# anrieff/fray

Measured on AMD Instinct MI355X. Metric: Mrays/s (closest-hit + shadow rays) at 1920x1080, 64spp path trace, higher is better.
Workload: dtype f64

## Files before the change

### fray_amd/abi.py

```python
import ctypes as C

i32, u32, i64, u64, f32, f64 = C.c_int32, C.c_uint32, C.c_int64, C.c_uint64, C.c_float, C.c_double
P = C.POINTER

ABI_VERSION = 3

OK, E_ARG, E_PARSE, E_NODEVICE, E_UNSUPPORTED, E_NOMEM, E_HIP, E_CANCELLED = 0, -1, -2, -3, -4, -5, -6, -7
GEOM_PLANE, GEOM_SPHERE, GEOM_CUBE, GEOM_MESH, GEOM_CSG = range(5)
TEX_CHECKER, TEX_BITMAP, TEX_BUMP, TEX_FRESNEL = range(4)
SHADER_CONST, SHADER_LAMBERT, SHADER_PHONG, SHADER_REFL, SHADER_REFR, SHADER_LAYERED = range(6)
LIGHT_POINT, LIGHT_RECT = range(2)
MODE_PRIMARY_ID, MODE_RENDER = 0, 1
FRAME_STATS = 1
OPTION_NAMES = ("pt_lanes", "pt_budget_mib", "speculate_fans", "fused_whitted_max", "fp_contract", "seed_table_mib", "skip_null_segments",
                "segment_planes", "certified_segments")
FIGURE_NAMES = ("contracted_launches", "shadow_segments", "segment_plane_nodes", "certified_segments_eligible", "shadow_segments_certified",
                "shadow_nodes_skipped", "seed_table_bytes", "seed_launches", "seed_planes_reused", "batch_lanes", "whitted_path",
                "pt_budget_effective_mib", "scene_updates", "scene_update_bytes", "arena_bytes", "fans_filed", "fan_children",
                "fan_children_looked_up", "fans_given_up")


class Transform(C.Structure):
    _fields_ = [("offset", f64 * 3), ("m", f64 * 9), ("invM", f64 * 9)]

# ... 137 lines not shown
    _fields_ = [("seed", u32), ("spp", i32), ("sample_first", i32), ("rng_skip", i32), ("flags", i32), ("_pad", i32),
                ("keys", C.c_void_p)]


class Adaptive(C.Structure):
    _fields_ = [("min_spp", i32), ("_pad", i32), ("threshold", f64), ("err_floor", f64), ("rungs", i32), ("_pad2", i32),
                ("samples", u64)]


ACCUM_CHANNELS = 4


class Samples(C.Structure):
    _fields_ = [("sample_first", i32), ("sample_count", i32), ("samples_done", i32), ("_pad", i32)]


class SamplesMap(C.Structure):
    _fields_ = [("samples", u64), ("count_min", i32), ("count_max", i32)]


class SampleMap(C.Structure):
    _fields_ = [("tolerance", C.c_float), ("lum_floor", C.c_float), ("min_count", i32), ("max_count", i32), ("max_add", i32), ("grow", i32),
                ("pixels", u64), ("samples", u64)]


class Denoise(C.Structure):
    _fields_ = [("levels", i32), ("demodulate", i32), ("sigma_luminance", C.c_float), ("sigma_normal", C.c_float),
                ("sigma_depth", C.c_float), ("sigma_albedo", C.c_float)]


FEAT_CHANNELS = 10
MOTION_CHANNELS = 8


class View(C.Structure):
    _fields_ = [("pos", f32 * 3), ("right", f32 * 3), ("up", f32 * 3), ("front", f32 * 3), ("tan_x", C.c_float), ("tan_y", C.c_float),
                ("width", i32), ("height", i32)]


class Temporal(C.Structure):
    _fields_ = [("demodulate", i32), ("max_history", i32), ("variance_history", i32), ("alpha_min", C.c_float), ("film_offset", C.c_float),
                ("plane_tolerance", C.c_float), ("normal_min_dot", C.c_float)]


class Change(C.Structure):
    _fields_ = [("radius", i32), ("gain", C.c_float)]


HISTORY_CHANNELS = 12
HISTORY_SPLIT_CHANNELS = 20


STRUCTS = {"frayhip_transform": Transform, "frayhip_geom_ref": GeomRef, "frayhip_node": Node,
           "frayhip_plane": Plane, "frayhip_sphere": Sphere, "frayhip_cube": Cube,
           "frayhip_csg": Csg, "frayhip_triangle": Triangle, "frayhip_kdnode": KDNode,
           "frayhip_mesh": Mesh, "frayhip_texture": Texture, "frayhip_shader": Shader,
           "frayhip_layer": Layer, "frayhip_light": Light, "frayhip_camera": Camera,
           "frayhip_settings": Settings, "frayhip_environment": Environment,
           "frayhip_scene_desc": SceneDesc, "frayhip_frame": Frame, "frayhip_stats": Stats,
           "frayhip_progress": Progress, "frayhip_progressive": Progressive,
           "frayhip_shade_request": ShadeRequest, "frayhip_adaptive": Adaptive, "frayhip_samples": Samples,
           "frayhip_view": View, "frayhip_samples_map": SamplesMap}

VP = C.c_void_p
SYMBOLS = {
    "frayhip_scene_parse": (C.c_int, [C.c_char_p, P(VP)]),
    "frayhip_host_scene_desc": (P(SceneDesc), [VP]),
    "frayhip_host_scene_free": (None, [VP]),
    "frayhip_init": (C.c_int, [C.c_int]),
    "frayhip_scene_create": (C.c_int, [P(SceneDesc), P(VP)]),
    "frayhip_scene_destroy": (None, [VP]),
    "frayhip_scene_set_view": (C.c_int, [VP, P(Camera), P(Settings)]),
    "frayhip_scene_update": (C.c_int, [VP, P(SceneDesc)]),
    "frayhip_transform_identity": (C.c_int, [P(Transform)]),
    "frayhip_transform_scale": (C.c_int, [P(Transform), f64, f64, f64]),
    "frayhip_transform_rotate": (C.c_int, [P(Transform), f64, f64, f64]),
    "frayhip_transform_translate": (C.c_int, [P(Transform), f64, f64, f64]),
    "frayhip_light_begin_frame": (C.c_int, [P(Light)]),
    "frayhip_shader_begin_frame": (C.c_int, [P(Shader)]),
    "frayhip_scene_set_option": (C.c_int, [VP, C.c_char_p, i64]),
    "frayhip_scene_get_option": (C.c_int, [VP, C.c_char_p, P(i64)]),
    "frayhip_scene_tight_gates": (C.c_int, [VP, C.c_int, P(i64), P(i64)]),
    "frayhip_scene_camera_skip": (C.c_int, [VP, C.c_int, P(i64), P(i64), P(i64), P(i64)]),
    "frayhip_render": (C.c_int, [VP, P(Frame), VP, VP, VP, P(Stats)]),
    "frayhip_render_device": (C.c_int, [VP, P(Frame), VP, VP, VP, VP, P(Stats)]),
    "frayhip_render_progressive": (C.c_int, [VP, P(Frame), P(Progressive), VP, VP, VP, P(Stats)]),
    "frayhip_render_device_progressive": (C.c_int, [VP, P(Frame), P(Progressive), VP, VP, VP, VP, P(Stats)]),
    "frayhip_render_adaptive": (C.c_int, [VP, P(Frame), P(Adaptive), VP, VP, VP, P(Stats)]),
    "frayhip_render_device_adaptive": (C.c_int, [VP, P(Frame), P(Adaptive), VP, VP, VP, VP, P(Stats)]),
    "frayhip_render_samples": (C.c_int, [VP, P(Frame), P(Samples), P(Progressive), VP, VP, VP, P(Stats)]),
    "frayhip_render_samples_device": (C.c_int, [VP, P(Frame), P(Samples), P(Progressive), VP, VP, VP, VP, P(Stats)]),
    "frayhip_render_components": (C.c_int, [VP, P(Frame), P(Samples), P(Progressive), VP, VP, VP, VP, VP, VP, P(Stats)]),
    "frayhip_render_components_device": (C.c_int, [VP, P(Frame), P(Samples), P(Progressive), VP, VP, VP, VP, VP, VP, VP, P(Stats)]),
    "frayhip_render_samples_map": (C.c_int, [VP, P(Frame), P(SamplesMap), VP, VP, VP, VP, VP, P(Stats)]),
    "frayhip_render_samples_map_device": (C.c_int, [VP, P(Frame), P(SamplesMap), VP, VP, VP, VP, VP, VP, P(Stats)]),
    "frayhip_render_components_map": (C.c_int, [VP, P(Frame), P(SamplesMap), VP, VP, VP, VP, VP, VP, VP, VP, P(Stats)]),
    "frayhip_render_components_map_device": (C.c_int, [VP, P(Frame), P(SamplesMap), VP, VP, VP, VP, VP, VP, VP, VP, VP, P(Stats)]),
    "frayhip_sample_map_defaults": (C.c_int, [P(SampleMap)]),
    "frayhip_sample_map": (C.c_int, [C.c_int, C.c_int, VP, VP, P(SampleMap), VP, P(Stats)]),
    "frayhip_sample_map_device": (C.c_int, [C.c_int, C.c_int, VP, VP, P(SampleMap), VP, VP, P(Stats)]),
    "frayhip_sample_map_pair": (C.c_int, [C.c_int, C.c_int, VP, VP, VP, P(SampleMap), VP, P(Stats)]),
    "frayhip_sample_map_pair_device": (C.c_int, [C.c_int, C.c_int, VP, VP, VP, P(SampleMap), VP, VP, P(Stats)]),
    "frayhip_render_features": (C.c_int, [VP, P(Frame), C.c_int, VP, P(Stats)]),
    "frayhip_render_features_device": (C.c_int, [VP, P(Frame), C.c_int, VP, VP, P(Stats)]),
    "frayhip_render_features_motion": (C.c_int, [VP, P(Frame), C.c_int, P(Transform), C.c_int, VP, VP, P(Stats)]),
    "frayhip_render_features_motion_device": (C.c_int, [VP, P(Frame), C.c_int, P(Transform), C.c_int, VP, VP, VP, P(Stats)]),
    "frayhip_denoise_defaults": (C.c_int, [P(Denoise)]),
    "frayhip_denoise": (C.c_int, [C.c_int, C.c_int, VP, VP, VP, P(Denoise), VP, P(Stats)]),
    "frayhip_denoise_device": (C.c_int, [C.c_int, C.c_int, VP, VP, VP, P(Denoise), VP, VP, P(Stats)]),
    "frayhip_denoise_signal": (C.c_int, [C.c_int, C.c_int, VP, VP, VP, P(Denoise), VP, P(Stats)]),
    "frayhip_denoise_signal_device": (C.c_int, [C.c_int, C.c_int, VP, VP, VP, P(Denoise), VP, VP, P(Stats)]),
    "frayhip_view_from_camera": (C.c_int, [P(Camera), C.c_int, C.c_int, P(View)]),
    "frayhip_temporal_defaults": (C.c_int, [P(Temporal)]),
    "frayhip_temporal_accumulate": (C.c_int, [C.c_int, C.c_int, VP, VP, P(View), VP, P(Temporal), VP, VP, VP, P(Stats)]),
    "frayhip_temporal_accumulate_device": (C.c_int, [C.c_int, C.c_int, VP, VP, P(View), VP, P(Temporal), VP, VP, VP, VP, P(Stats)]),
    "frayhip_temporal_accumulate_motion": (C.c_int, [C.c_int, C.c_int, VP, VP, VP, P(View), VP, P(Temporal), VP, VP, VP, P(Stats)]),
    "frayhip_temporal_accumulate_motion_device": (C.c_int, [C.c_int, C.c_int, VP, VP, VP, P(View), VP, P(Temporal), VP, VP, VP, VP, P(Stats)]),
    "frayhip_temporal_accumulate_split": (C.c_int, [C.c_int, C.c_int, VP, VP, VP, VP, P(View), VP, P(Temporal), P(Temporal), VP, VP, VP, VP, VP, P(Stats)]),
    "frayhip_temporal_accumulate_split_device": (C.c_int, [C.c_int, C.c_int, VP, VP, VP, VP, P(View), VP, P(Temporal), P(Temporal), VP, VP, VP, VP, VP, VP,
                                                           P(Stats)]),
    "frayhip_change_defaults": (C.c_int, [P(Change)]),
    "frayhip_change_frame": (C.c_int, [C.c_int, C.c_int, VP, VP, VP, P(Change), VP, P(Stats)]),
    "frayhip_change_frame_device": (C.c_int, [C.c_int, C.c_int, VP, VP, VP, P(Change), VP, VP, P(Stats)]),
    "frayhip_temporal_accumulate_adaptive": (C.c_int, [C.c_int, C.c_int, VP, VP, VP, VP, P(View), VP, P(Temporal), VP, VP, VP, P(Stats)]),
    "frayhip_temporal_accumulate_adaptive_device": (C.c_int, [C.c_int, C.c_int, VP, VP, VP, VP, P(View), VP, P(Temporal), VP, VP, VP, VP, P(Stats)]),
    "frayhip_temporal_accumulate_split_adaptive": (C.c_int, [C.c_int, C.c_int, VP, VP, VP, VP, VP, VP, P(View), VP, P(Temporal), P(Temporal), VP, VP, VP, VP,
                                                             VP, P(Stats)]),
    "frayhip_temporal_accumulate_split_adaptive_device": (C.c_int, [C.c_int, C.c_int, VP, VP, VP, VP, VP, VP, P(View), VP, P(Temporal), P(Temporal), VP, VP,
                                                                    VP, VP, VP, VP, P(Stats)]),
    "frayhip_camera_rays": (C.c_int, [VP, i64, VP, C.c_int, VP, VP]),
    "frayhip_camera_rays_device": (C.c_int, [VP, i64, VP, C.c_int, VP, VP, VP]),
    "frayhip_trace_rays": (C.c_int, [VP, i64, VP, VP, C.c_int, VP, VP, VP, P(Stats)]),
    "frayhip_trace_rays_device": (C.c_int, [VP, i64, VP, VP, C.c_int, VP, VP, VP, VP, P(Stats)]),
    "frayhip_visible": (C.c_int, [VP, i64, VP, VP, C.c_int, VP, P(Stats)]),
    "frayhip_visible_device": (C.c_int, [VP, i64, VP, VP, C.c_int, VP, VP, P(Stats)]),
    "frayhip_shade_rays": (C.c_int, [VP, i64, VP, VP, P(ShadeRequest), VP, P(Stats)]),
    "frayhip_shade_rays_device": (C.c_int, [VP, i64, VP, VP, P(ShadeRequest), VP, VP, P(Stats)]),
    "frayhip_bucket_count": (C.c_int, [C.c_int, C.c_int, C.c_int, C.c_int]),
    "frayhip_pack_buckets_device": (C.c_int, [VP, VP, C.c_int, C.c_int, C.c_int, C.c_int, C.c_int, VP]),
    "frayhip_unpack_buckets_device": (C.c_int, [VP, VP, C.c_int, C.c_int, C.c_int, C.c_int, C.c_int, VP]),
    "frayhip_bucket_xy": (C.c_int, [C.c_int, C.c_int, C.c_int, C.POINTER(C.c_int), C.POINTER(C.c_int)]),
    "frayhip_comm_available": (C.c_int, []),
    "frayhip_comm_library": (C.c_char_p, []),
    "frayhip_comm_unique_id": (C.c_int, [VP]),
    "frayhip_comm_create": (C.c_int, [VP, C.c_int, C.c_int, P(VP)]),
    "frayhip_comm_from_nccl": (C.c_int, [VP, C.c_int, C.c_int, P(VP)]),
    "frayhip_comm_ranks": (C.c_int, [VP]),
    "frayhip_comm_destroy": (None, [VP]),
    "frayhip_gather_buckets": (C.c_int, [VP, VP, C.c_int, C.c_int, C.c_int, C.c_int, VP]),
    "frayhip_to_rgb32": (C.c_int, [VP, VP, C.c_int]),
    "frayhip_save_bmp": (C.c_int, [C.c_char_p, VP, C.c_int, C.c_int]),
    "frayhip_debug_rng": (C.c_int, [u32, C.c_int, VP, VP, VP, C.c_int]),
    "frayhip_debug_libm": (C.c_int, [C.c_int, VP, VP, VP, VP, VP]),
    "frayhip_debug_arith": (C.c_int, [C.c_int, C.c_int, VP, VP, VP]),
    "frayhip_last_error": (C.c_char_p, []),
    "frayhip_abi_version": (C.c_int, []),
    "frayhip_sizeof": (C.c_int, [C.c_char_p]),
}


def bind(lib):
    for name, (res, args) in SYMBOLS.items():
        fn = getattr(lib, name)
        fn.restype = res
        fn.argtypes = args
    return lib
# ... 1 lines not shown
```

### fray_amd/csrc/capi.hip

```cpp
#include <hip/hip_runtime.h>

#include <algorithm>
#include <chrono>
#include <cstddef>
#include <cmath>
#include <cstring>
#include <string>
#include <vector>
#include <functional>
#include <cstdlib>


#include "entry_support.hpp"
#include "dev_rng.hpp"
#include "dev_pack.hpp"
#include "scene_arena.hpp"

namespace {

using frayhip_detail::set_error;

void put3(double* o, const double* p) { o[0] = p[0]; o[1] = p[1]; o[2] = p[2]; }
}

// ... 148 lines not shown
    if (T.d) (void)hipFree(T.d);
    T.d = nullptr;
    T.bytes = 0;
    T.valid.clear();
    T.serving = false;
}

void seed_table_begin(frayhip_scene* sc, const DFrame& F, int nItems, int spp)
{
    SeedTable& T = sc->seedTab;
    if (!sc->seedTableCapBytes) { seed_table_free(sc); T.keyed = false; return; }
    if (nItems <= 0 || spp <= 0) return;
    const int32_t key[7] = {F.W, F.H, F.BW, F.BH, F.bucketFirst, F.bucketStride, F.nBuckets};
    const size_t planeBytes = (size_t)nItems * sizeof(uint32_t);
    if (!T.keyed || memcmp(key, T.key, sizeof key) != 0 || F.seed != T.seed || nItems != T.nItems) {
        memcpy(T.key, key, sizeof key);
        T.seed = F.seed; T.nItems = nItems; T.keyed = true; T.noGrow = false;
        T.valid.assign(T.bytes / planeBytes, 0);
    }
    const size_t need = (size_t)spp * planeBytes;
    if (need > sc->seedTableCapBytes) return;
    if (T.valid.size() < (size_t)spp) {
        if (T.noGrow) return;
        uint32_t* d = nullptr;
        if (hipMalloc((void**)&d, need) != hipSuccess) {
            (void)hipGetLastError();
            seed_table_free(sc);
            T.noGrow = true;
            return;
        }
        size_t held = 0;
        for (size_t s = 0; s < T.valid.size(); s++) if (T.valid[s]) held = s + 1;
        if (held && hipMemcpy(d, T.d, held * planeBytes, hipMemcpyDeviceToDevice) != hipSuccess) { (void)hipGetLastError(); std::fill(T.valid.begin(), T.valid.end(), (unsigned char)0); }
        if (T.d) (void)hipFree(T.d);
        T.d = d;
        T.bytes = need;
        T.valid.resize((size_t)spp, 0);
    }
    T.serving = true;
}

hipEvent_t pool_event(std::vector<hipEvent_t>& pool, size_t i)
{
    while (pool.size() <= i) {
        hipEvent_t e = nullptr;
        hipError_t rc = hipEventCreate(&e);
        if (rc != hipSuccess) { set_error(std::string("hipEventCreate: ") + hipGetErrorString(rc)); return nullptr; }
        pool.push_back(e);
    }
    return pool[i];
}

int bad(const char* who, const std::string& why)
{
    set_error(std::string(who) + ": " + why);
    return FRAYHIP_E_ARG;
}
int unsupported(const char* who, const std::string& why)
{
    set_error(std::string(who) + ": " + why);
    return FRAYHIP_E_UNSUPPORTED;
}

int frame_spp(const frayhip_scene* s)
{
    int spp = s->settings.wantAA ? 5 : 1;
    if (s->camera.dof) spp = std::max(spp, s->camera.numDOFSamples);
    if (s->settings.gi) spp = std::max(spp, s->settings.numPaths);
    return spp;
}

DScene frame_scene(const frayhip_scene* s)
{
    const frayhip_settings& set = s->settings;
    DScene S = s->S;
    S.ambient[0] = set.ambientLight[0]; S.ambient[1] = set.ambientLight[1]; S.ambient[2] = set.ambientLight[2];
    S.maxTraceDepth = set.maxTraceDepth;
    S.gi = set.gi;
    S.saturation = set.saturation;
    S.skipNullSegments = s->skipNullSegments ? 1 : 0;
    S.segmentPlanes = s->segmentPlanes ? 1 : 0;
    S.certifiedSegments = (s->certifiedSegments && s->segmentPlanes && S.segCertAll) ? 1 : 0;
    if (!s->cameraSkip) S.nCamSkip = 0;
    return S;
}

DFrame frame_record(const frayhip_scene* s, int bucketFirst, int bucketStride, uint32_t seed)
{
    DFrame F = frame_grid(s->settings.frameWidth, s->settings.frameHeight);
    F.bucketStride = bucketStride > 0 ? bucketStride : 1;
    F.bucketFirst = bucketFirst;
    F.nBuckets = frayhip_bucket_count(F.W, F.H, F.bucketFirst, F.bucketStride);
    F.spp = frame_spp(s);
    F.seed = seed;
    F.jitter = (s->camera.dof || s->settings.gi) ? 1 : 0;
    return F;
}

int check_bucket_range(const char* who, int nBuckets) { return nBuckets < 0 ? bad(who, "bad bucket_first / bucket_stride") : FRAYHIP_OK; }
int check_pixel_cap(const char* who, int nBuckets)
{
    if ((long long)nBuckets * 2304 > (1ll << 30)) return unsupported(who, "more than 2^30 pixels in one call (shard the frame with bucket_first / bucket_stride)");
    return FRAYHIP_OK;
}
int refuse_stereo(const char* who, const frayhip_scene* s) { return s->camera.stereoSeparation > 0 ? unsupported(who, "stereo frames are not supported") : FRAYHIP_OK; }
int refuse_long_generators(const char* who, const frayhip_scene* s, const char* by)
{
    if (s->settings.gi && s->settings.maxTraceDepth >= 0 && long_generators(s->settings.maxTraceDepth))
        return unsupported(who, std::string("path tracing with maxTraceDepth >= 20 (generators past 227 words) is not supported by ") + by);
    return FRAYHIP_OK;
}

frayhip_stats finish_stats(frayhip_scene* sc, const DStats* blocks, int nBlocks, size_t nTraceEvents, size_t nShadowEvents, std::chrono::steady_clock::time_point t0)
{
    frayhip_stats o{};
    for (int k = 0; k < nBlocks; k++) {
        const DStats& d = blocks[k];
        o.closest_rays += d.closest; o.shadow_rays += d.shadow; o.node_tests += d.node; o.kd_inner_visits += d.kdInner; o.leaf_refs += d.leafRefs;
        o.tri_tests += d.tri; o.prim_tests += d.prim; o.smooth_hits += d.smooth; o.samples += d.samples; o.texture_fetches += d.tex;
    }
    float ms = 0;
    (void)hipEventElapsedTime(&ms, sc->evA, sc->evB);
    o.ms_kernels = ms;
    auto sumEvents = [](const std::vector<hipEvent_t>& pool, size_t n) {
        double t = 0;
        for (size_t i = 0; i + 1 < n; i += 2) {
            float m2 = 0;
            (void)hipEventElapsedTime(&m2, pool[i], pool[i + 1]);
            t += m2;
        }
        return t;
    };
    o.ms_trace = sumEvents(sc->evPool, nTraceEvents);
    o.trace_launches = nTraceEvents / 2;
    o.ms_shadow = sumEvents(sc->evPoolShadow, nShadowEvents);
    o.shadow_launches = nShadowEvents / 2;
    o.ms_total = std::chrono::duration<double, std::milli>(std::chrono::steady_clock::now() - t0).count();
    return o;
}

}

struct SceneEdit {
    frayhip_arena::ArenaFacts F;
    std::vector<frayhip_arena::ArenaTable> tables;
    std::vector<frayhip_arena::ArenaMeshTables> meshTables;
    std::vector<int64_t> texelOffset;
    std::vector<unsigned char> host;
    std::vector<int64_t> hostOff;
    int32_t counts[11];
    int64_t nTexels;
    std::vector<frayhip_geom_ref> geoms;
    std::vector<frayhip_csg> csgs;
    std::vector<frayhip_mesh> meshes;
    std::vector<frayhip_texture> textures;
    frayhip_environment environment;
};

namespace frayhip_detail {
const DNode* host_nodes(const frayhip_scene* s) { return (const DNode*)(s->edit->host.data() + s->edit->hostOff[s->edit->F.tNodes]); }
}

namespace {

using frayhip_detail::kStatsBytes;
using frayhip_detail::grid_for;
// ... 168 lines not shown
    sc->whittedNeedsRecursion = F.whittedNeedsRecursion != 0;
    sc->lightDraws = F.lightDraws != 0;
    sc->lightSampleCount = F.lightSampleCount;
    sc->specFanMax = F.specFanMax;
}

}

extern "C" {

int frayhip_init(int device_id)
{
    int n = 0;
    hipError_t e = hipGetDeviceCount(&n);
    if (e != hipSuccess || n <= 0) { set_error("frayhip_init: no HIP device available"); return FRAYHIP_E_NODEVICE; }
    if (device_id < 0 || device_id >= n) { set_error("frayhip_init: bad device id"); return FRAYHIP_E_ARG; }
    HIP_TRY(hipSetDevice(device_id));
    return FRAYHIP_OK;
}

int frayhip_scene_create(const frayhip_scene_desc* desc, frayhip_scene** out)
{
    if (!desc || !out) { set_error("frayhip_scene_create: null argument"); return FRAYHIP_E_ARG; }
    if (desc->abi_version != FRAYHIP_ABI_VERSION) { set_error("frayhip_scene_create: ABI version mismatch"); return FRAYHIP_E_ARG; }
    const frayhip_scene_desc& d = *desc;
    {
        const std::string why = validate_desc(d);
        if (!why.empty()) { set_error(why); return FRAYHIP_E_ARG; }
    }
    {
        std::vector<int> levels(d.n_csgs, 0);
        std::function<int(int, int)> depth = [&](int i, int guard) -> int {
            if (guard > d.n_csgs) return 1 << 20;
            if (levels[i]) return levels[i];
            int m = 1;
            for (int side = 0; side < 2; side++) {
                const frayhip_geom_ref& g = d.geoms[side == 0 ? d.csgs[i].left : d.csgs[i].right];
                if (g.kind == FRAYHIP_GEOM_CSG) m = std::max(m, 1 + depth(g.index, guard + 1));
            }
            return levels[i] = m;
        };
        for (int i = 0; i < d.n_csgs; i++)
            if (depth(i, 0) > FRAY_CSG_DEPTH) {
                set_error("frayhip_scene_create: CSG operands nested more than " + std::to_string(FRAY_CSG_DEPTH) + " levels deep are not implemented on the device path");
                return FRAYHIP_E_UNSUPPORTED;
            }
    }
    frayhip_arena::ArenaBuilt B;
    frayhip_arena::arena_build(d, B);
    frayhip_scene* sc = new frayhip_scene();
    commit_facts(sc, B.F);
    if (hipMalloc(&sc->d_arena, B.host.size() ? B.host.size() : 256) != hipSuccess) {
        set_error("frayhip_scene_create: hipMalloc failed (no device?)");
        delete sc;
        return FRAYHIP_E_NODEVICE;
    }
    {
        unsigned char* const base = (unsigned char*)sc->d_arena;
        std::vector<unsigned char*> stage(B.tables.size());
        std::vector<const unsigned char*> addr(B.tables.size());
        for (size_t t = 0; t < B.tables.size(); t++) { stage[t] = B.host.data() + B.tables[t].off; addr[t] = base + B.tables[t].off; }
        frayhip_arena::arena_place(B.F, B.meshTables.data(), B.texelOffset.data(), stage.data(), addr.data(), sc->S);
    }
    hipError_t e = hipMemcpy(sc->d_arena, B.host.data(), B.host.size(), hipMemcpyHostToDevice);
    if (e != hipSuccess) { set_error(std::string("frayhip_scene_create: upload failed: ") + hipGetErrorString(e)); (void)hipFree(sc->d_arena); delete sc; return FRAYHIP_E_NODEVICE; }
    sc->arena_bytes = B.host.size();
    sc->edit = make_scene_edit(d, B);
    sc->camera = d.camera;
    sc->settings = d.settings;
    if (hipMalloc((void**)&sc->d_stats, kStatsBytes) != hipSuccess || hipMalloc((void**)&sc->d_qmeta, 3 * FRAY_PT_LANES * sizeof(QMeta)) != hipSuccess ||
        hipEventCreate(&sc->evA) != hipSuccess || hipEventCreate(&sc->evB) != hipSuccess || !create_lanes(sc)) {
        set_error("frayhip_scene_create: could not allocate the per-scene device state");
        frayhip_scene_destroy(sc);
        return FRAYHIP_E_NOMEM;
    }
    if (const char* e = getenv("FRAYHIP_PT_LANES")) { long v = atol(e); if (v >= 1 && v <= FRAY_PT_LANES) sc->ptLanes = (int)v; }
    if (const char* e = getenv("FRAYHIP_SPECULATE_FANS")) sc->speculateFans = atol(e) != 0;
    if (const char* e = getenv("FRAYHIP_FP_CONTRACT")) sc->fpContract = atol(e) == 1;
    if (const char* e = getenv("FRAYHIP_SKIP_NULL_SEGMENTS")) sc->skipNullSegments = atol(e) != 0;
    if (const char* e = getenv("FRAYHIP_SEGMENT_PLANES")) sc->segmentPlanes = atol(e) != 0;
    if (const char* e = getenv("FRAYHIP_CERTIFIED_SEGMENTS")) sc->certifiedSegments = atol(e) != 0;
    if (const char* e = getenv("FRAYHIP_TIGHT_GATES")) sc->tightGates = atol(e) != 0;
    if (const char* e = getenv("FRAYHIP_CAMERA_SKIP")) sc->cameraSkip = atol(e) != 0;
    if (const char* e = getenv("FRAYHIP_FUSED_WHITTED_MAX")) { long v = atol(e); if (v >= 0 && v <= 1024) sc->fusedWhittedMax = (int)v; }
    if (const char* e = getenv("FRAYHIP_CSG_LANES")) { long v = atol(e); if (v >= 1 && v <= FRAY_PT_LANES) sc->csgLanes = (int)v; }
    if (const char* e = getenv("FRAYHIP_SEED_TABLE_MIB")) { long v = atol(e); if (v >= 0 && v <= (1 << 20)) sc->seedTableCapBytes = (size_t)v << 20; }
    if (const char* e = getenv("FRAYHIP_PT_BUDGET_MIB")) { long v = atol(e); if (v >= 1 && v <= (1 << 20)) { sc->ptBudgetBytes = (size_t)v << 20; sc->ptBudgetEff = 0; } }
    *out = sc;
    return FRAYHIP_OK;
}

int frayhip_scene_get_option(frayhip_scene* s, const char* name, int64_t* value)
{
    if (!s || !name || !value) { set_error("frayhip_scene_get_option: null argument"); return FRAYHIP_E_ARG; }
    const std::string n(name);
    if (n == "pt_lanes") *value = s->ptLanes;
    else if (n == "pt_budget_mib") *value = (int64_t)(s->ptBudgetBytes >> 20);
    else if (n == "speculate_fans") *value = s->speculateFans ? 1 : 0;
    else if (n == "fp_contract") *value = s->fpContract ? 1 : 0;
    else if (n == "contracted_launches") *value = s->lastContracted;
    else if (n == "skip_null_segments") *value = s->skipNullSegments ? 1 : 0;
    else if (n == "shadow_segments") *value = s->lastShadowSegments;
    else if (n == "segment_planes") *value = s->segmentPlanes ? 1 : 0;
    else if (n == "segment_plane_nodes") *value = s->S.nSegNodes;
    else if (n == "certified_segments") *value = s->certifiedSegments ? 1 : 0;
    else if (n == "certified_segments_eligible") *value = s->S.segCertAll;
    else if (n == "shadow_segments_certified") *value = s->lastShadowCertified;
    else if (n == "shadow_nodes_skipped") *value = s->lastShadowNodesSkipped;
    else if (n == "seed_table_mib") *value = (int64_t)(s->seedTableCapBytes >> 20);
    else if (n == "seed_table_bytes") *value = (int64_t)s->seedTab.bytes;
    else if (n == "seed_launches") *value = s->lastSeedLaunches;
    else if (n == "seed_planes_reused") *value = s->lastSeedReused;
    else if (n == "batch_lanes") *value = s->lastBatchLanes;
    else if (n == "whitted_path") *value = s->lastWhittedPath;
    else if (n == "fused_whitted_max") *value = s->fusedWhittedMax;
    else if (n == "pt_budget_effective_mib") *value = (int64_t)(frayhip_detail::work_budget(s) >> 20);
    else if (n == "scene_updates") *value = s->sceneUpdates;
    else if (n == "scene_update_bytes") *value = s->sceneUpdateBytes;
    else if (n == "arena_bytes") *value = (int64_t)s->arena_bytes;
    else if (n == "fans_filed") *value = s->lastFans[0];
    else if (n == "fan_children") *value = s->lastFans[1];
    else if (n == "fan_children_looked_up") *value = s->lastFans[2];
    else if (n == "fans_given_up") *value = s->lastFans[3];
    else { set_error("frayhip_scene_get_option: unknown option " + n); return FRAYHIP_E_ARG; }
    return FRAYHIP_OK;
}

int frayhip_scene_set_option(frayhip_scene* s, const char* name, int64_t value)
{
    if (!s || !name) { set_error("frayhip_scene_set_option: null argument"); return FRAYHIP_E_ARG; }
    if (s->rendering) { set_error("frayhip_scene_set_option: the scene is rendering a frame"); return FRAYHIP_E_ARG; }
    const std::string n(name);
    if (n == "pt_lanes") {
        if (value < 1 || value > FRAY_PT_LANES) { set_error("frayhip_scene_set_option: pt_lanes must be 1.." + std::to_string(FRAY_PT_LANES)); return FRAYHIP_E_ARG; }
        s->ptLanes = (int)value;
    } else if (n == "pt_budget_mib") {
        if (value < 1 || value > (1 << 20)) { set_error("frayhip_scene_set_option: pt_budget_mib must be 1..1048576"); return FRAYHIP_E_ARG; }
        s->ptBudgetBytes = (size_t)value << 20;
        s->ptBudgetEff = 0;
    } else if (n == "speculate_fans") {
        if (value != 0 && value != 1) { set_error("frayhip_scene_set_option: speculate_fans must be 0 or 1"); return FRAYHIP_E_ARG; }
        s->speculateFans = value != 0;
    } else if (n == "fused_whitted_max") {
        if (value < 0 || value > 1024) { set_error("frayhip_scene_set_option: fused_whitted_max must be 0..1024"); return FRAYHIP_E_ARG; }
        s->fusedWhittedMax = (int)value;
    } else if (n == "fp_contract") {
        if (value != 0 && value != 1) { set_error("frayhip_scene_set_option: fp_contract must be 0 or 1"); return FRAYHIP_E_ARG; }
        s->fpContract = value != 0;
    } else if (n == "seed_table_mib") {
        if (value < 0 || value > (1 << 20)) { set_error("frayhip_scene_set_option: seed_table_mib must be 0..1048576"); return FRAYHIP_E_ARG; }
        s->seedTableCapBytes = (size_t)value << 20;
        if (s->seedTab.bytes > s->seedTableCapBytes) { frayhip_detail::seed_table_free(s); s->seedTab.keyed = false; }
    } else if (n == "skip_null_segments") {
        if (value != 0 && value != 1) { set_error("frayhip_scene_set_option: skip_null_segments must be 0 or 1"); return FRAYHIP_E_ARG; }
        s->skipNullSegments = value != 0;
    } else if (n == "segment_planes") {
        if (value != 0 && value != 1) { set_error("frayhip_scene_set_option: segment_planes must be 0 or 1"); return FRAYHIP_E_ARG; }
        s->segmentPlanes = value != 0;
    } else if (n == "certified_segments") {
        if (value != 0 && value != 1) { set_error("frayhip_scene_set_option: certified_segments must be 0 or 1"); return FRAYHIP_E_ARG; }
        s->certifiedSegments = value != 0;
    } else {
        set_error("frayhip_scene_set_option: unknown option " + n);
        return FRAYHIP_E_ARG;
    }
    return FRAYHIP_OK;
}

int frayhip_scene_tight_gates(frayhip_scene* s, int enable, int64_t* enabled, int64_t* eligible)
{
    if (!s) { set_error("frayhip_scene_tight_gates: null scene"); return FRAYHIP_E_ARG; }
    if (enable < -1 || enable > 1) { set_error("frayhip_scene_tight_gates: enable must be -1, 0 or 1"); return FRAYHIP_E_ARG; }
    if (enable >= 0 && s->rendering) { set_error("frayhip_scene_tight_gates: the scene is rendering a frame"); return FRAYHIP_E_ARG; }
    if (enable >= 0) s->tightGates = enable != 0;
    if (enabled) *enabled = s->tightGates ? 1 : 0;
    if (eligible) *eligible = s->edit->F.nTightGates;
    return FRAYHIP_OK;
}

int frayhip_scene_camera_skip(frayhip_scene* s, int enable, int64_t* enabled, int64_t* eligible, int64_t* skipped, int64_t* waves)
{
    if (!s) { set_error("frayhip_scene_camera_skip: null scene"); return FRAYHIP_E_ARG; }
    if (enable < -1 || enable > 1) { set_error("frayhip_scene_camera_skip: enable must be -1, 0 or 1"); return FRAYHIP_E_ARG; }
    if (enable >= 0 && s->rendering) { set_error("frayhip_scene_camera_skip: the scene is rendering a frame"); return FRAYHIP_E_ARG; }
    if (enable >= 0) s->cameraSkip = enable != 0;
    if (enabled) *enabled = s->cameraSkip ? 1 : 0;
    if (eligible) *eligible = s->edit->F.nCamSkip;
    if (skipped) *skipped = s->lastCameraSkipped;
    if (waves) *waves = s->lastCameraWaves;
    return FRAYHIP_OK;
}

int frayhip_scene_set_view(frayhip_scene* s, const frayhip_camera* camera, const frayhip_settings* settings)
{
    if (!s) { set_error("frayhip_scene_set_view: null scene"); return FRAYHIP_E_ARG; }
    if (s->rendering) { set_error("frayhip_scene_set_view: the scene is rendering a frame"); return FRAYHIP_E_ARG; }
    if (settings && (settings->frameWidth <= 0 || settings->frameHeight <= 0)) { set_error("frayhip_scene_set_view: bad frame size"); return FRAYHIP_E_ARG; }
    if (camera) s->camera = *camera;
    if (settings) s->settings = *settings;
    return FRAYHIP_OK;
}

int frayhip_scene_update(frayhip_scene* s, const frayhip_scene_desc* desc)
{
    if (!s || !desc) { set_error("frayhip_scene_update: null argument"); return FRAYHIP_E_ARG; }
    if (s->rendering) { set_error("frayhip_scene_update: the scene is rendering a frame"); return FRAYHIP_E_ARG; }
    if (desc->abi_version != FRAYHIP_ABI_VERSION) { set_error("frayhip_scene_update: ABI version mismatch"); return FRAYHIP_E_ARG; }
    const frayhip_scene_desc& d = *desc;
    SceneEdit& E = *s->edit;
    if (const char* what = fixed_part_differs(E, d)) {
        set_error(std::string("frayhip_scene_update: ") + what + " differs from the description the scene was created from (only nodes, primitives, shaders, layers, lights and texture parameters can be edited)");
        return FRAYHIP_E_ARG;
    }
    {
        const std::string why = validate_editable(d, "frayhip_scene_update");
        if (!why.empty()) { set_error(why); return FRAYHIP_E_ARG; }
    }
    std::vector<unsigned char> next(E.host);
    frayhip_arena::ArenaFacts F = E.F;
    std::vector<unsigned char*> tab(E.tables.size());
    std::vector<const unsigned char*> addr(E.tables.size());
    for (size_t t = 0; t < E.tables.size(); t++) {
        tab[t] = E.hostOff[t] >= 0 ? next.data() + E.hostOff[t] : nullptr;
        addr[t] = (const unsigned char*)s->d_arena + E.tables[t].off;
    }
    frayhip_arena::arena_update(d, E.meshTables.data(), F, tab.data());
    DScene S = s->S;
    frayhip_arena::arena_place(F, E.meshTables.data(), E.texelOffset.data(), tab.data(), addr.data(), S);
    long long bytes = 0;
    for (int32_t t : frayhip_arena::arena_editable_tables(F)) {
        if (!E.tables[t].bytes) continue;
        HIP_TRY(hipMemcpy((unsigned char*)s->d_arena + E.tables[t].off, tab[t], E.tables[t].bytes, hipMemcpyHostToDevice));
        bytes += (long long)E.tables[t].bytes;
    }
    E.host.swap(next);
    E.F = F;
    commit_facts(s, F);
    s->S = S;
    s->sceneUpdates++;
    s->sceneUpdateBytes = bytes;
    return FRAYHIP_OK;
}

void frayhip_scene_destroy(frayhip_scene* s)
{
    if (!s) return;
    delete s->edit;
    if (s->d_arena) (void)hipFree(s->d_arena);
    if (s->d_work) (void)hipFree(s->d_work);
    frayhip_detail::seed_table_free(s);
    if (s->d_stats) (void)hipFree(s->d_stats);
    if (s->d_motionTab) (void)hipFree(s->d_motionTab);
    if (s->d_qmeta) (void)hipFree(s->d_qmeta);
    if (s->evA) (void)hipEventDestroy(s->evA);
    if (s->evB) (void)hipEventDestroy(s->evB);
    if (s->evLaneStart) (void)hipEventDestroy(s->evLaneStart);
    for (int k = 0; k < FRAY_PT_LANES; k++) {
        if (s->evResolved[k]) (void)hipEventDestroy(s->evResolved[k]);
        if (s->laneStream[k]) (void)hipStreamDestroy(s->laneStream[k]);
    }
    for (auto e : s->evPool) (void)hipEventDestroy(e);
    for (auto e : s->evPoolShadow) (void)hipEventDestroy(e);
    delete s;
}


namespace {
int render_dispatch(frayhip_scene* s, const frayhip_frame* f, float* d_rgb, int32_t* d_hit_id, double* d_hit_dist, hipStream_t stream, frayhip_stats* st,
                    const frayhip_detail::Progress* prog)
{
    if (s->rendering) { set_error("frayhip_render: the scene is already rendering a frame (a render call from inside a progress callback?)"); return FRAYHIP_E_ARG; }
    frayhip_detail::Busy busy(s, stream, false);
    return frayhip_detail::for_flag_word(frayhip_detail::flag_word(s, (f->flags & FRAYHIP_FRAME_STATS) != 0), [&](auto w) {
        return frayhip_detail::render_impl<decltype(w)::value>(s, f, d_rgb, d_hit_id, d_hit_dist, stream, st, prog, nullptr);
    });
// ... 153 lines not shown
```

### fray_amd/csrc/dev_scene.hpp

```cpp
#pragma once
#include <stdint.h>
#include "frayhip.h"
#include "dev_tricert.hpp"
#include "dev_segcert.hpp"
#include "dev_gatecert.hpp"

#ifdef __HIP_DEVICE_COMPILE__
#define FRAY_RO __attribute__((address_space(4)))
#else
#define FRAY_RO
#endif

#define FRAY_CSG_MAX 30
#ifndef FRAY_CSG_DEPTH
#define FRAY_CSG_DEPTH 16
#endif

#define FRAY_KD_LDS_STACK 16
#define FRAY_KD_MAX_DEPTH 72

struct DXform { double off[3]; double m[9]; double inv[9]; };

struct DTri;
struct DNode {
    DXform T;
    int32_t geomKind, geomIndex, shader, bumpTex;
    int32_t xfClass;
    int32_t tlTris;
    int32_t tlCulling;
    int32_t xfIdentity;
    double bmin[3], bmax[3];
    const FRAY_RO DTri* tlPtr;
    double boxMax;
    int32_t gated;
    int32_t segNode;
};
struct DNodeX {
    double bminE[3], bmaxE[3];
    double cc[3], ch[3], cM;
    int32_t csgBox, padX;
};

struct DPlane { double limit, height; };
struct DSphere { double O[3]; double R; };
struct DCube { double O[3]; double halfSide; };
struct DCsg { int32_t op, leftKind, leftIndex, rightKind, rightIndex, leftGeom, rightGeom, flat; };

struct DTri {
    double g[3];
    double A[3];
    double N[3];
    double AC[3];
    double AB[3];
    int32_t index;
    int32_t pad;
};

struct DTriAttr {
    double nA[3], nB[3], nC[3];
    double tA[2], tB[2], tC[2];
    double dNdx[3], dNdy[3];
};

struct alignas(16) DKd {
    union {
        double split;
        struct { int32_t triBegin, triCount; };
    };
    int32_t child0;
    int32_t meta;
};
struct DKdBox { double lo[3], hi[3]; };

struct DMesh {
    double bmin[3], bmax[3];
    const FRAY_RO DTri* tris;
    const FRAY_RO DTriAttr* attrs;
    const FRAY_RO DKd* kd;
    const FRAY_RO DKdBox* kdBox;
    const FRAY_RO int32_t* refs;
    const FRAY_RO DTri* ltris;
    int32_t nTris, hasKd, smooth, culling, hasUV, pad;
    double boxMax;
    const FRAY_RO DTri32* ltris32;
    double ref[3];
};

struct DTexture {
    int32_t kind, width, height, pad;
    float color1[3], color2[3];
    double scaling, bumpIntensity, ior;
    const FRAY_RO float* texels;
};

struct DShader {
    int32_t kind, texture;
    float color[3], specularColor[3], mult[3];
    int32_t numSamples;
    double exponent, specularMultiplier, glossiness, deflectionScaling, ior;
    int32_t layerBegin, layerCount;
    int32_t usesUV, pad;
};

struct DLayer { int32_t shader, texture; float opacity[3]; int32_t pad; };

struct DLight {
    int32_t kind, xSubd, ySubd, pad;
    float color[3], power;
    double pos[3];
    DXform T;
    double center[3];
    double area;
    double areaXsize, areaYsize;
};

struct DEnv {
    int32_t present, loaded;
    int32_t width[6], height[6];
    const FRAY_RO float* face[6];
};

struct DCamera {
    double topLeft[3], topRight[3], bottomLeft[3];
    double frontDir[3], upDir[3], rightDir[3], pos[3];
    double w, h, apertureSize, focalPlaneDist, stereoSeparation;
    float leftMask[3], rightMask[3];
    int32_t dof, pad;
};

#define FRAY_MAX_GATES 8
#define FRAY_GATE_MIN_TRIS 6
struct DGate { double lo[3], hi[3]; float cf[3], hf[3]; float Mf; int32_t exact; float guard; int32_t nDirs; float nf[FRAY_GATE_MAX_DIRS][3]; };

#define FRAY_CAMSKIP_MAX 16
struct DCamSkip { float cf[3], hf[3]; float Mf, guard; float nf[FRAY_GATE_MAX_DIRS][3]; int32_t nDirs, node; };

struct DScene {
    const FRAY_RO DNode* nodes;
    const FRAY_RO DNodeX* nodesX;
    const FRAY_RO DGate* gates;
    int32_t nGates, gatesExact;
    const FRAY_RO DPlane* planes;
    const FRAY_RO DSphere* spheres;
    const FRAY_RO DCube* cubes;
    const FRAY_RO DCsg* csgs;
    const FRAY_RO DMesh* meshes;
    const FRAY_RO DShader* shaders;
    const FRAY_RO DLayer* layers;
    const FRAY_RO DTexture* textures;
    const FRAY_RO DLight* lights;
    DEnv env;
    int32_t nNodes, nLights;
    float probPickLight;
    float ambient[3];
    int32_t maxTraceDepth, gi;
    float saturation;
    const FRAY_RO DSegPlane* segPlanes;
    const FRAY_RO uint32_t* segNodeMasks;
    int32_t nSegPlanes, nSegNodes;
    int32_t segmentPlanes;
    int32_t skipNullSegments;
    int32_t segCertAll;
    int32_t certifiedSegments;
    const FRAY_RO DCamSkip* camSkip;
    int32_t nCamSkip, padCamSkip;
};

struct DFrame {
    int32_t W, H, BW, BH;
    int32_t bucketFirst, bucketStride, nBuckets , spp;
    uint32_t seed;
    int32_t jitter;
};

struct DStats {
    unsigned long long closest, shadow, node, kdInner, leafRefs, tri, prim, smooth, samples, tex, rngOverflow;
#ifdef FRAY_STAMPS
    unsigned long long stamp[24];
    unsigned long long stampLanes[24];
#endif
};
struct DCursors { unsigned int v[8][32]; };
```

### fray_amd/csrc/dev_shade.hpp

```cpp
#pragma once
#include "dev_math.hpp"
#include "dev_rng.hpp"
#include "dev_scene.hpp"
#include "dev_trace.hpp"

enum { RF_DIFFUSE = 2 };

struct HitInfo {
    V3 ip, norm, dNdx, dNdy;
    double u, v;
};

FD void prim_attributes(const DScene& S, int kind, int index, V3 ipl, int code, double l2, double l3, bool needUV, bool needBump, V3& nl, HitInfo& info)
{
    if (kind == 0) {
        nl = v3(0, 1, 0);
        info.u = ipl.x;
        info.v = ipl.z;
    } else if (kind == 1) {
        const FRAY_RO DSphere& Sp = S.spheres[index];
        nl = normalized(ipl - ld3(Sp.O));
        if (needUV) {
            info.u = ((atan2(nl.z, nl.x) / FRAY_PI * 180.0) + 180.0) / 360.0;
            info.v = 1 - ((asin(nl.y) / FRAY_PI * 180.0) + 90) / 180.0;
        }
    } else if (kind == 2) {
        const int ax = code >> 1;
        const double sg = (code & 1) ? +1.0 : -1.0;
        nl = v3(ax == 0 ? sg : 0.0, ax == 1 ? sg : 0.0, ax == 2 ? sg : 0.0);
        if (ax == 0) { info.u = ipl.y; info.v = ipl.z; }
        else if (ax == 1) { info.u = ipl.x; info.v = ipl.z; }
        else { info.u = ipl.x; info.v = ipl.y; }
    } else {
        const FRAY_RO DMesh& M = S.meshes[index];
        const FRAY_RO DTriAttr* A = M.attrs + code;
        if (M.smooth) {
            V3 nA = ld3(A->nA), nB = ld3(A->nB), nC = ld3(A->nC);
            nl = normalized(nA + (nB - nA) * l2 + (nC - nA) * l3);
        } else {
            nl = ld3(M.tris[code].g);
        }
        if (M.hasUV) {
            info.u = A->tA[0] + (A->tB[0] - A->tA[0]) * l2 + (A->tC[0] - A->tA[0]) * l3;
            info.v = A->tA[1] + (A->tB[1] - A->tA[1]) * l2 + (A->tC[1] - A->tA[1]) * l3;
        }
        if (needBump) {
            info.dNdx = ld3(A->dNdx);
            info.dNdy = ld3(A->dNdy);
        }
    }
}

template <int ST, bool BARY = false, bool ANY_UV = false>
FD void finalize_hit(const DScene& S, const HitT<ST>& h, V3 o, V3 d, bool needUV, HitInfo& info)
{
    const FRAY_RO DNode& N = S.nodes[h.node];
    needUV = needUV && (ANY_UV || tex_variant(ST));
    const bool needBump = tex_variant(ST) && N.bumpTex >= 0;
    V3 ls = mulM(o - ld3(N.T.off), N.T.inv);
    V3 ldir = normalized(mulM(d, N.T.inv));
    V3 ipl = ls + ldir * h.t;
    V3 nl;
    info.dNdx = v3(0, 0, 0);
    info.dNdy = v3(0, 0, 0);
    info.u = 0; info.v = 0;
    bool done = false;
    if constexpr ((ST & 2) != 0) {
        if (N.geomKind == 2) {
            ipl = h.ipl;
            prim_attributes(S, 2, N.geomIndex, ipl, h.tri, 0, 0, needUV, needBump, nl, info);
            done = true;
        } else if (N.geomKind == 4) {
            ipl = h.ipl;
            prim_attributes(S, h.leafKind, h.leafIndex, ipl, h.tri, h.l2, h.l3, needUV, needBump, nl, info);
            done = true;
        }
    }
    if (!done) {
        double l2 = h.l2, l3 = h.l3;
        if (BARY && N.geomKind == 3) {
            const FRAY_RO DMesh& M = S.meshes[N.geomIndex];
            if (M.smooth || M.hasUV) tri_bary(M.tris + h.tri, ls, ldir, l2, l3);
        }
        prim_attributes(S, N.geomKind, N.geomIndex, ipl, h.tri, l2, l3, needUV, needBump, nl, info);
    }
    info.ip = mulM(ipl, N.T.m) + ld3(N.T.off);
    info.norm = normalized(mulM(nl, N.T.m));
}

template <int ST>
FD C3 texel(const FRAY_RO DTexture& T, int x, int y, Cnt& c)
{
    bump<ST>(c.tex);
    if (T.width <= 0 || x < 0 || x >= T.width || y < 0 || y >= T.height) return c3(0, 0, 0);
    return ldc(T.texels + 3 * ((long long)x + (long long)y * T.width));
}
FD void wrap_texel(const FRAY_RO DTexture& T, double u, double v, int& ix, int& iy)
{
    ix = int(floor(u * T.scaling * T.width));
    iy = int(floor(v * T.scaling * T.height));
    ix %= T.width;
    iy %= T.height;
    if (ix < 0) ix += T.width;
    if (iy < 0) iy += T.height;
}
FD float fresnel_schlick(V3 i, V3 n, float ior)
{
    float q = (1.0f - ior) / (1.0f + ior);
    float f = (float)((double)q * (double)q);
    float NdotI = (float)-dot(n, i);
    return f + (1.0f - f) * powf(1.0f - NdotI, 5.0f);
}
template <int ST>
FD C3 texture_sample(const DScene& S, int t, V3 rayDir, const HitInfo& info, Cnt& c)
{
    if (!tex_variant(ST)) return c3(1, 1, 1);
    const FRAY_RO DTexture& T = S.textures[t];
    if (T.kind == 0) {
        int ix = int(floor(info.u * T.scaling) / 5.0);
        int iy = int(floor(info.v * T.scaling) / 5.0);
        return ((ix + iy) % 2 == 0) ? ldc(T.color1) : ldc(T.color2);
    }
    if (T.kind == 1) {
        int ix, iy;
        wrap_texel(T, info.u, info.v, ix, iy);
        return texel<ST>(T, ix, iy, c);
    }
    if (T.kind == 3) {
        V3 n;
        double myIor;
        if (dot(rayDir, info.norm) < 0) { n = info.norm; myIor = T.ior; }
        else { n = -info.norm; myIor = 1.0 / T.ior; }
        float f = fresnel_schlick(rayDir, n, (float)myIor);
        return c3(f, f, f);
    }
    return c3(0, 0, 0);
}
template <int ST>
FD void apply_bump(const DScene& S, int nodeIdx, HitInfo& info, Cnt& c)
{
    if (!tex_variant(ST)) return;
    int bt = S.nodes[nodeIdx].bumpTex;
    if (bt < 0) return;
    const FRAY_RO DTexture& T = S.textures[bt];
    if (T.kind != 2) return;
    int ix, iy;
    wrap_texel(T, info.u, info.v, ix, iy);
    C3 t = texel<ST>(T, ix, iy, c);
    float dx = (float)(t.r * T.bumpIntensity);
    float dy = (float)(t.g * T.bumpIntensity);
    info.norm = info.norm + ((double)dx * info.dNdx + (double)dy * info.dNdy) * T.bumpIntensity;
    info.norm = normalized(info.norm);
}

template <int ST>
FD C3 environment(const DScene& S, V3 dir, Cnt& c)
{
    if (!tex_variant(ST) || !S.env.present || !S.env.loaded) return c3(0, 0, 0);
    double maxVal = fabs(dir.x);
    int dim = 0;
    if (fabs(dir.y) > maxVal) { dim = 1; maxVal = fabs(dir.y); }
    if (fabs(dir.z) > maxVal) dim = 2;
    bool positive = comp(dir, dim) > 0;
    V3 on = dir * (1.0 / fabs(comp(dir, dim)));
    int face = (positive ? 3 : 0) + dim;
    double sx, sy;
    switch (face) {
        case 0: sx = on.z; sy = -on.y; break;
        case 3: sx = -on.z; sy = -on.y; break;
        case 1: sx = on.x; sy = -on.z; break;
        case 4: sx = on.x; sy = on.z; break;
        case 2: sx = on.x; sy = on.y; break;
        default: sx = on.x; sy = -on.y; break;
    }
    int W = S.env.width[face], H = S.env.height[face];
    int ix = (int)(((sx + 1) / 2) * W);
    int iy = (int)(((sy + 1) / 2) * H);
    bump<ST>(c.tex);
    if (ix < 0 || ix >= W || iy < 0 || iy >= H) return c3(0, 0, 0);
    return ldc(S.env.face[face] + 3 * ((long long)ix + (long long)iy * W));
}

FD int light_num_samples(const FRAY_RO DLight& L) { return L.kind == 0 ? 1 : L.xSubd * L.ySubd; }
FD C3 light_color(const FRAY_RO DLight& L) { return ldc(L.color) * L.power; }
template <class G>
FD void light_nth_sample(const FRAY_RO DLight& L, int idx, V3 shadePos, G& tab, V3& samplePos, C3& color)
{
    if (L.kind == 0) {
        samplePos = ld3(L.pos);
        color = ldc(L.color) * L.power;
        return;
    }
    int col = idx % L.xSubd;
    int row = idx / L.xSubd;
    double cellW = L.areaXsize;
    double cellH = L.areaYsize;
    double x0 = col * cellW;
    double y0 = row * cellH;
    double p_x = x0 + cellW * rng_float(tab);
    double p_y = y0 + cellH * rng_float(tab);
    V3 pl = v3(p_x - 0.5, 0, p_y - 0.5);
    V3 sp = mulM(shadePos - ld3(L.T.off), L.T.inv);
    if (sp.y > 0) {
        color = c3(0, 0, 0);
    } else {
        float cw = float(fray_div(dot(v3(0, -1, 0), sp), length(sp)));
        color = ldc(L.color) * L.power * (float)L.area * cw;
    }
    samplePos = mulM(pl, L.T.m) + ld3(L.T.off);
}
FD double light_solid_angle(const FRAY_RO DLight& L, V3 ip)
{
    if (L.kind == 0) return 0;
    double q = lengthSqr(ip - ld3(L.center));
    return fray_div(L.area, 1.0 < q ? q : 1.0);
}

template <int ST, class G>
FD C3 shade_direct(const DScene& S, const FRAY_RO DShader& sh, V3 rayDir, const HitInfo& info, G& tab, bool phong, Cnt& c)
{
    C3 diffuse = ldc(sh.color);
    if (sh.texture >= 0) diffuse = diffuse * texture_sample<ST>(S, sh.texture, rayDir, info, c);
    C3 result = diffuse * ldc(S.ambient);
    const int nl = S.nLights;
    for (int li = 0; li < nl; li++) {
        const FRAY_RO DLight& L = S.lights[li];
        const int ns = light_num_samples(L);
        C3 sum = c3(0, 0, 0);
        for (int k = 0; k < ns; k++) {
            C3 lc;
            V3 lp;
            light_nth_sample(L, k, info.ip, tab, lp, lc);
            double d2 = lengthSqr(info.ip - lp);
            V3 wl = normalized(lp - info.ip);
            V3 n = faceforward(rayDir, info.norm);
            float cosN = (float)dot(wl, n);
            float lam = (float)(cosN / d2);
            lam = lam > 0.0f ? lam : 0.0f;
            if (visible<ST>(S, info.ip + n * 1e-6, lp, c)) {
                C3 r = diffuse * lc * lam;
                if (phong) {
                    V3 wi = -wl;
                    V3 rr = reflect(wi, n);
                    double cosV = dot(-rayDir, rr);
                    if (cosV > 0)
                        r = r + lc / (float)d2 * ldc(sh.specularColor) * (float)pow(cosV, sh.exponent) * (float)sh.specularMultiplier;
                }
                sum = sum + r;
            }
        }
        result = result + sum / (float)ns;
    }
    return result;
}

template <class G>
FD V3 hemisphere_sample(G& tab, V3 norm)
{
    double u = rng_double(tab);
    double v = rng_double(tab);
    double theta = 2 * FRAY_PI * u;
    double sp, cp, st, ct;
    fray_acos_sincos(2 * v - 1, &sp, &cp);
    fray_sincos(theta, &st, &ct);
    V3 dir = v3(sp * ct, cp, sp * st);
    if (dot(dir, norm) > 0) return dir;
    return -dir;
}
FD C3 brdf_eval(const FRAY_RO DShader& sh, const HitInfo& x, V3 w_out)
{
    if (sh.kind == 1) {
        double dd = dot(x.norm, w_out);
        float cosTerm = (float)(0.0 < dd ? dd : 0.0);
        return ldc(sh.color) * (float)fray_div(cosTerm, FRAY_PI);
    }
    if (sh.kind == 3 || sh.kind == 4) return c3(0, 0, 0);
    return c3(1, 0, 0);
}
FD int spawn_words(const FRAY_RO DShader& sh) { return sh.kind == 1 ? 4 : 0; }

struct PathRay { V3 o, d; int depth; unsigned flags; };

template <class G>
FD void spawn_ray(const FRAY_RO DShader& sh, const HitInfo& x, const PathRay& w_in, G& tab, PathRay& w_out, C3& brdf, float& pdf)
{
    w_out = w_in;
    if (sh.kind == 1) {
        w_out.depth = w_in.depth + 1;
        w_out.o = x.ip + x.norm * 1e-6;
        w_out.d = hemisphere_sample(tab, x.norm);
        w_out.flags |= RF_DIFFUSE;
        double dd = dot(x.norm, w_out.d);
        float cosTerm = (float)(0.0 < dd ? dd : 0.0);
        brdf = ldc(sh.color) * (float)fray_div(cosTerm, FRAY_PI);
        pdf = (float)(1 / (2 * FRAY_PI));
        return;
    }
    if (sh.kind == 3) {
        V3 n = faceforward(w_in.d, x.norm);
        w_out.depth = w_in.depth + 1;
        w_out.o = x.ip + n * 1e-6;
        w_out.d = reflect(w_in.d, x.norm);
        w_out.flags &= ~(unsigned)RF_DIFFUSE;
        brdf = ldc(sh.mult) * 1e9f;
        pdf = 1e9f;
        return;
    }
    if (sh.kind == 4) {
        V3 n = faceforward(w_in.d, x.norm);
        double myIor = dot(n, x.norm) > 0 ? 1.0 / sh.ior : sh.ior / 1.0;
        V3 refr = refract(w_in.d, n, myIor);
        if (!(refr.x == 0 && refr.y == 0 && refr.z == 0)) {
            w_out.o = x.ip - n * 1e-6;
            w_out.d = refr;
            w_out.depth = w_in.depth + 1;
            w_out.flags &= ~(unsigned)RF_DIFFUSE;
            brdf = ldc(sh.mult) * 1e9f;
            pdf = 1e9f;
        } else {
            w_out.depth = w_in.depth + 1;
            brdf = c3(0, 0, 0);
            pdf = 1.0f;
        }
        return;
    }
    w_out.depth = w_in.depth + 1;
    brdf = c3(1, 0, 0);
    pdf = 1;
}

template <class GR, class GT>
FD bool nee_prepare(const DScene& S, V3 rayDir, const HitInfo& info, C3 pm, const FRAY_RO DShader& sh, GR& rnd, GT& tab, V3& a, V3& b, C3& contrib, bool skipNull)
{
    if (S.nLights == 0) return false;
    int lightIdx = rng_int0(rnd, S.nLights - 1);
    const FRAY_RO DLight& L = S.lights[lightIdx];
    V3 x = info.ip;
    double solidAngle = light_solid_angle(L, x);
    if (solidAngle == 0) return false;
    int randSample = rng_int0(rnd, light_num_samples(L) - 1);
    V3 pl;
    C3 unused;
    light_nth_sample(L, randSample, x, tab, pl, unused);
    if (skipNull && (sh.kind == 3 || sh.kind == 4)) return false;
    a = x + info.norm * 1e-6;
    b = pl;
    C3 Le = light_color(L);
    V3 w_out = normalized(pl - x);
    C3 brdfAtPoint = brdf_eval(sh, info, w_out);
    if (intensity(brdfAtPoint) == 0) { contrib = c3(0, 0, 0); return !skipNull; }
    float probHitLightArea = (float)fray_rcp(solidAngle);
    float probPickThisLight = S.probPickLight;
    float chooseLightProb = probHitLightArea * probPickThisLight;
    contrib = Le * pm * brdfAtPoint / chooseLightProb;
    if (skipNull && (__float_as_uint(contrib.r) | __float_as_uint(contrib.g) | __float_as_uint(contrib.b)) == 0u) return false;
    return true;
}
```

### fray_amd/csrc/dev_trace.hpp

```cpp
#pragma once
#ifndef FRAY_IDENTITY_SKIP
#define FRAY_IDENTITY_SKIP 1
#endif
#ifndef FRAY_FILTER_STRAIGHT
#define FRAY_FILTER_STRAIGHT 1
#endif
#include "dev_math.hpp"
#include "dev_scene.hpp"
#include "dev_sort.hpp"
#define FRAY_CERT_SEQ() __builtin_amdgcn_sched_barrier(0)
#include "dev_boxcert.hpp"
#include "dev_misscert.hpp"
#include "dev_segcert.hpp"

#ifdef FRAY_LEAFSTAT
static __device__ unsigned long long g_leafStat[4];
#endif
struct Cnt {
    unsigned long long closest, shadow, node, kdInner, leafRefs, tri, prim, smooth, samples, tex;
    unsigned envelope;
};
template <int ST> FD void bump(unsigned long long& c, unsigned long long n = 1) { if (ST & 1) c += n; }
constexpr bool kd_variant(int st) { return (st & 6) != 0; }
constexpr bool tex_variant(int st) { return (st & 14) != 0; }
constexpr bool identity_variant(int st) { return FRAY_IDENTITY_SKIP && (st & 14) == 0; }
constexpr bool tight_variant(int st) { return FRAY_ARITH == 0 && (st & 15) == 0; }

struct HitRec {
    int node;
    int tri;
    double dist;
    double t;
    double l2, l3;
};
struct HitRecX : HitRec {
    V3 ipl;
    int leafKind, leafIndex;
};
template <int ST> struct HitOf { typedef HitRec type; };
template <> struct HitOf<2> { typedef HitRecX type; };
template <> struct HitOf<3> { typedef HitRecX type; };
template <int ST> using HitT = typename HitOf<ST>::type;

struct Box6 { double lox, loy, loz, hix, hiy, hiz; };

struct LocalRay { V3 s, d, rd; int cls; bool haveRd, dirOk; double rmax, sMax; };


FD bool box_inside(const Box6& b, V3 v)
{
    return b.lox - 1e-6 <= v.x && v.x <= b.hix + 1e-6 && b.loy - 1e-6 <= v.y && v.y <= b.hiy + 1e-6 &&
           b.loz - 1e-6 <= v.z && v.z <= b.hiz + 1e-6;
}

struct BoxDim { bool rej, hit; };
FD BoxDim box_dim(double sd, double dd, double rd, double lo, double hi, double su, double du, double lou, double hiu,
                  double sv, double dv, double lov, double hiv)
{
    BoxDim r;
    r.rej = (dd < 0 && sd < lo) | (dd > 0 && sd > hi);
    const bool skip = fabs(dd) < 1e-9;
    const double d1 = (lo - sd) * rd;
    const bool near = !(d1 < 0);
    const double x1 = su + du * d1, y1 = sv + dv * d1;
    const bool hitN = (lou <= x1) & (x1 <= hiu) & (lov <= y1) & (y1 <= hiv);
    const double d2 = (hi - sd) * rd;
    const bool far = !(d2 < 0);
    const double x2 = su + du * d2, y2 = sv + dv * d2;
    const bool hitF = far & (lou <= x2) & (x2 <= hiu) & (lov <= y2) & (y2 <= hiv);
    r.hit = !r.rej & !skip & near & (hitN | hitF);
    return r;
}

FD bool box_test_pre(const Box6& b, const Box6& be, V3 s, V3 d, V3 rd)
{
    bool res = be.lox <= s.x && s.x <= be.hix && be.loy <= s.y && s.y <= be.hiy && be.loz <= s.z && s.z <= be.hiz;
    bool alive = !res;
    if (!__any(alive)) return res;
    BoxDim a = box_dim(s.x, d.x, rd.x, b.lox, b.hix, s.y, d.y, b.loy, b.hiy, s.z, d.z, b.loz, b.hiz);
    res |= alive & a.hit;
    alive &= !a.rej & !a.hit;
    if (!__any(alive)) return res;
    a = box_dim(s.y, d.y, rd.y, b.loy, b.hiy, s.x, d.x, b.lox, b.hix, s.z, d.z, b.loz, b.hiz);
    res |= alive & a.hit;
    alive &= !a.rej & !a.hit;
    if (!__any(alive)) return res;
    a = box_dim(s.z, d.z, rd.z, b.loz, b.hiz, s.x, d.x, b.lox, b.hix, s.y, d.y, b.loy, b.hiy);
    res |= alive & a.hit;
    return res;
}

FD bool box_test(const Box6& b, V3 s, V3 d, V3 rd)
{
    bool res = box_inside(b, s);
    bool alive = !res;
    BoxDim a = box_dim(s.x, d.x, rd.x, b.lox, b.hix, s.y, d.y, b.loy, b.hiy, s.z, d.z, b.loz, b.hiz);
    res |= alive & a.hit;
    alive &= !a.rej & !a.hit;
    if (!__any(alive)) return res;
    a = box_dim(s.y, d.y, rd.y, b.loy, b.hiy, s.x, d.x, b.lox, b.hix, s.z, d.z, b.loz, b.hiz);
    res |= alive & a.hit;
    alive &= !a.rej & !a.hit;
    if (!__any(alive)) return res;
    a = box_dim(s.z, d.z, rd.z, b.loz, b.hiz, s.x, d.x, b.lox, b.hix, s.y, d.y, b.loy, b.hiy);
    res |= alive & a.hit;
    return res;
}

FD void box_set_hi(Box6& b, int axis, double v) { b.hix = axis == 0 ? v : b.hix; b.hiy = axis == 1 ? v : b.hiy; b.hiz = axis == 2 ? v : b.hiz; }
// ... 653 lines not shown
        tri = h.code;
        t = h.dist;
        l2 = h.l2; l3 = h.l3;
        lo->kind = h.leafKind; lo->index = h.leafIndex;
        return true;
    }
    double gamma;
    if (N.tlTris > 0) {
        prepare_ray<ST>(lr);
        Box6 box;
        box.lox = N.bmin[0]; box.loy = N.bmin[1]; box.loz = N.bmin[2];
        box.hix = N.bmax[0]; box.hiy = N.bmax[1]; box.hiz = N.bmax[2];
        bool rootHit;
        if constexpr (kd_variant(ST)) {
            TState st;
            rootHit = box_test_cert(box, lr, cert_ray(lr.rmax, lr.sMax, lr.dirOk, N.boxMax), st);
        } else {
            const FRAY_RO DNodeX& X = S.nodesX[nodeIndex];
            Box6 be;
            be.lox = X.bminE[0]; be.loy = X.bminE[1]; be.loz = X.bminE[2];
            be.hix = X.bmaxE[0]; be.hiy = X.bmaxE[1]; be.hiz = X.bmaxE[2];
            rootHit = box_test_pre(box, be, ls, ld, lr.rd);
        }
        STAMP(2);
        if (!rootHit) return false;
        gamma = 1e99;
        bool found = false;
        const int n = N.tlTris, culling = N.tlCulling;
        const FRAY_RO DTri* tris = N.tlPtr;
        for (int i = 0; i < n; i++)
            if (tri_test<ST>(tris + i, culling, ls, ld, gamma, l2, l3, c)) { found = true; tri = i; }
        STAMP(3);
        if (!found) return false;
    } else if (!kd_variant(ST)) {
        return false;
    } else if (!mesh_intersect<ST>(S.meshes[N.geomIndex], lr, gamma, tri, l2, l3, c)) return false;
    ipl = ls + ld * gamma;
    t = gamma;
    return true;
}

template <int ST>
FD bool node_intersect(const DScene& S, int i, V3 o, V3 d, LocalRay& lr, double& dist, double& t, int& tri, double& l2, double& l3, V3* iplOut, LeafOut* lo, Cnt& c)
{
    bump<ST>(c.node);
    const FRAY_RO DNode& N = S.nodes[i];
    if (N.xfClass != lr.cls) {
        bool done = false;
        if constexpr (identity_variant(ST)) {
#if FRAY_ARITH
            if (N.xfIdentity) { lr.s = o; lr.d = d; done = true; }
#else
            const bool zeros = o.x == 0 || o.y == 0 || o.z == 0 || d.x == 0 || d.y == 0 || d.z == 0;
            if (N.xfIdentity && !__any(zeros)) { lr.s = o; lr.d = normalized(d); done = true; }
#endif
        }
        if (!done) {
            lr.s = mulM(o - ld3(N.T.off), N.T.inv);
            lr.d = normalized(mulM(d, N.T.inv));
        }
        lr.cls = N.xfClass;
        lr.haveRd = false;
    }
    STAMP(1);
    V3 ipl;
    const bool hit = geom_intersect<ST>(S, N, i, lr, ipl, t, tri, l2, l3, lo, c);
    STAMP(5);
    if (!hit) return false;
    if constexpr ((ST & 2) != 0) { if (iplOut) *iplOut = ipl; }
    V3 ipw;
    if constexpr (identity_variant(ST)) {
#if FRAY_ARITH
        if (N.xfIdentity) { dist = t; STAMP(6); return true; }
#endif
        ipw = N.xfIdentity ? ipl : mulM(ipl, N.T.m) + ld3(N.T.off);
    } else {
        ipw = mulM(ipl, N.T.m) + ld3(N.T.off);
    }
    dist = length(o - ipw);
    STAMP(6);
    return true;
}

template <int ST>
FD bool light_intersect(const FRAY_RO DLight& L, V3 o, V3 d, double& dist, Cnt& c)
{
    if (L.kind == 0) return false;
    bump<ST>(c.prim);
    V3 ls = mulM(o - ld3(L.T.off), L.T.inv);
    V3 ldir = normalized(mulM(d, L.T.inv));
    if (ls.y >= 0) return false;
    if (ldir.y <= 0) return false;
    double travelByY = fabs(ls.y);
    double unitTravel = fabs(ldir.y);
    double scaling = fray_div(travelByY, unitTravel);
    V3 ip = ls + ldir * scaling;
    if (fabs(ip.x) > 0.5 || fabs(ip.z) > 0.5) return false;
    ip = mulM(ip, L.T.m) + ld3(L.T.off);
    dist = length(o - ip);
    return true;
}

FD void light_record(const FRAY_RO DLight& L, V3 o, V3 d, V3& ip, V3& norm)
{
    V3 ls = mulM(o - ld3(L.T.off), L.T.inv);
    V3 ldir = normalized(mulM(d, L.T.inv));
    double scaling = fray_div(fabs(ls.y), fabs(ldir.y));
    ip = mulM(ls + ldir * scaling, L.T.m) + ld3(L.T.off);
    norm = normalized(mulM(v3(0, -1, 0), L.T.m));
}

template <int ST, bool CAMSKIP = false>
FD void closest_hit(const DScene& S, V3 o, V3 d, HitT<ST>& best, Cnt& c, bool gateFree = false, uint32_t skipNodes = 0u)
{
    bump<ST>(c.closest);
    best.node = -1;
    best.tri = -1;
    best.dist = 1e99;
    best.t = 0; best.l2 = 0; best.l3 = 0;
    const int nn = S.nNodes;
    LocalRay lr;
    lr.cls = -1;
    lr.haveRd = false;
    for (int i = 0; i < nn; i++) {
        double dist, t, l2 = 0, l3 = 0;
        int tri = -1;
        if constexpr (CAMSKIP) { if (i < 32 && ((skipNodes >> i) & 1u)) continue; }
        if constexpr (!(ST & 1)) { if (S.nodes[i].gated) { if (gateFree) continue; } }
        if constexpr ((ST & 2) != 0) {
            V3 ipl;
            LeafOut lo{0, 0};
            if (node_intersect<ST>(S, i, o, d, lr, dist, t, tri, l2, l3, &ipl, &lo, c) && dist < best.dist) {
                best.node = i; best.tri = tri; best.dist = dist; best.t = t; best.l2 = l2; best.l3 = l3;
                best.ipl = ipl; best.leafKind = lo.kind; best.leafIndex = lo.index;
            }
        } else if (node_intersect<ST>(S, i, o, d, lr, dist, t, tri, l2, l3, nullptr, nullptr, c) && dist < best.dist) {
            best.node = i; best.tri = tri; best.dist = dist; best.t = t; best.l2 = l2; best.l3 = l3;
        }
    }
    if ((ST & 1) && best.node >= 0) {
        const FRAY_RO DNode& W = S.nodes[best.node];
        if (W.geomKind == 3 && S.meshes[W.geomIndex].smooth) c.smooth++;
    }
    STAMP(6);
    const int nl = S.nLights;
    for (int i = 0; i < nl; i++) {
        double dist;
        if (light_intersect<ST>(S.lights[i], o, d, dist, c) && dist < best.dist) {
            best.node = -2 - i;
            best.dist = dist;
        }
    }
    STAMP(7);
}

FD uint32_t segment_skip_nodes(const DScene& S, V3 a, V3 b, bool live)
{
    const int nP = S.segmentPlanes ? S.nSegPlanes : 0;
    if (nP <= 0) return 0u;
    const V3 e = b - a;
    const double m = seg_cert_scale(a.x, a.y, a.z, b.x, b.y, b.z, e.x, e.y, e.z);
    const lanes_t all = lanes(true);
    uint32_t certified = 0;
    for (int p = 0; p < nP; p++) {
        const FRAY_RO DSegPlane& P = S.segPlanes[p];
        if (lanes(!live || seg_same_side(P.N[0], P.N[1], P.N[2], P.k, P.t0, P.t1, m, a.x, a.y, a.z, b.x, b.y, b.z)) == all) certified |= 1u << p;
    }
    uint32_t skipNodes = 0;
    const int nS = S.nSegNodes;
    for (int j = 0; j < nS; j++)
        if ((S.segNodeMasks[j] & ~certified) == 0u) skipNodes |= 1u << j;
    return skipNodes;
}

FD uint32_t camera_skip_nodes(const DScene& S, V3 o, V3 d, bool live)
{
    const int nR = S.nCamSkip;
    if (nR <= 0) return 0u;
    const float dx = (float)d.x, dy = (float)d.y, dz = (float)d.z;
    const float dsum = fabsf(dx) + fabsf(dy) + fabsf(dz);
    const float ox = (float)o.x, oy = (float)o.y, oz = (float)o.z;
    const float omax = fmaxf(fmaxf(fabsf(ox), fabsf(oy)), fabsf(oz));
    const bool range = gate_ray_range(dsum, omax, ox + oy + oz);
    const lanes_t all = lanes(true);
    uint32_t skipNodes = 0;
    for (int r = 0; r < nR; r++) {
        const FRAY_RO DCamSkip& R = S.camSkip[r];
        bool miss = ray_surely_misses_box_f32(R.cf[0], R.cf[1], R.cf[2], R.hf[0], R.hf[1], R.hf[2], R.Mf, ox, oy, oz, dx, dy, dz, omax, dsum);
        miss = miss & gate_guard_f32(R, dx, dy, dz, dsum);
        miss = miss & range;
        if (lanes(!live || miss) == all) skipNodes |= 1u << R.node;
    }
    return skipNodes;
}

#ifdef __HIP__
#define FRAY_RCPF(x) __builtin_amdgcn_rcpf(x)
#else
#define FRAY_RCPF(x) (1.0f / (x))
#endif
template <bool TIGHT = false>
FD uint32_t ray_gate_class(const DScene& S, V3 o, V3 d)
{
    const int ng = S.nGates;
    if (ng == 0) return 0u;
    if constexpr (TIGHT) {
        if (S.gatesExact) {
            const float dx = (float)d.x, dy = (float)d.y, dz = (float)d.z;
            const float dsum = fabsf(dx) + fabsf(dy) + fabsf(dz);
            bool guarded = true, tight = false;
            for (int g = 0; g < ng; g++) {
                const FRAY_RO DGate& G = S.gates[g];
                if (G.nDirs) { guarded = guarded & gate_guard_f32(G, dx, dy, dz, dsum); tight = true; }
            }
            FRAY_CERT_SEQ();
            const float ox = (float)o.x, oy = (float)o.y, oz = (float)o.z;
            const float omax = fmaxf(fmaxf(fabsf(ox), fabsf(oy)), fabsf(oz));
            uint32_t first = 0;
            for (int g = ng - 1; g >= 0; g--) {
                const FRAY_RO DGate& G = S.gates[g];
                if (!ray_surely_misses_box_f32(G.cf[0], G.cf[1], G.cf[2], G.hf[0], G.hf[1], G.hf[2], G.Mf, ox, oy, oz, dx, dy, dz, omax, dsum)) first = (uint32_t)g + 1u;
            }
            if (tight) guarded = guarded & gate_ray_range(dsum, omax, ox + oy + oz);
            if (!guarded && !first) first = 1u;
            return !(omax < 1e9f) && !first ? 1u : first;
        }
    }
    const float ox = (float)o.x, oy = (float)o.y, oz = (float)o.z;
    if (S.gatesExact) {
        const float dx = (float)d.x, dy = (float)d.y, dz = (float)d.z;
        const float omax = fmaxf(fmaxf(fabsf(ox), fabsf(oy)), fabsf(oz)), dsum = fabsf(dx) + fabsf(dy) + fabsf(dz);
// ... 60 lines not shown
```

### fray_amd/csrc/kernels.hpp

```cpp
#pragma once
#include "dev_shade.hpp"
#include "dev_whitted.hpp"
#include "dev_queues.hpp"
#include <type_traits>

#ifndef FRAY_PRIMARY_WAVES
#define FRAY_PRIMARY_WAVES 5
#endif
#ifndef FRAY_WHITTED_WAVES
#define FRAY_WHITTED_WAVES 3
#endif
#ifndef FRAY_WHITTED_REFILL
#define FRAY_WHITTED_REFILL 64
#endif
#ifndef FRAY_CSG_WAVES
#define FRAY_CSG_WAVES 3
#endif
constexpr int waves_for(int st, int n) { return (st & 2) ? (FRAY_CSG_WAVES < n ? FRAY_CSG_WAVES : n) : ((st & 1) && n > 2 ? n - 1 : n); }
#ifndef FRAY_MT_EARLY
#define FRAY_MT_EARLY 160
#endif
#ifndef FRAY_WH_SHADE_WAVES
#define FRAY_WH_SHADE_WAVES 4
#endif
// ... 844 lines not shown
                ps.tab = ps.rnd;
                float ox = rng_float(ps.rnd), oy = rng_float(ps.rnd);
                double fx = (double)((float)x + ox), fy = (double)((float)y + oy);
                const int which = stereo ? 1 : 0;
                if (C.dof) dof_ray(C, fx, fy, ps.tab, ps.o, ps.d, which); else screen_ray(C, fx, fy, ps.o, ps.d, which);
                if (stereo) {
                    V3 ro, rd;
                    if (C.dof) dof_ray(C, fx, fy, ps.tab, ro, rd, 2); else screen_ray(C, fx, fy, ro, rd, 2);
                    SB.r[0][slot] = ro.x; SB.r[1][slot] = ro.y; SB.r[2][slot] = ro.z;
                    SB.r[3][slot] = rd.x; SB.r[4][slot] = rd.y; SB.r[5][slot] = rd.z;
                }
            } else {
                ps.rnd.j = SB.g[0][slot]; ps.rnd.a = SB.g[1][slot]; ps.rnd.b = SB.g[2][slot];
                ps.tab.j = SB.g[3][slot]; ps.tab.a = SB.g[4][slot]; ps.tab.b = SB.g[5][slot];
                ps.o = v3(SB.r[0][slot], SB.r[1][slot], SB.r[2][slot]);
                ps.d = v3(SB.r[3][slot], SB.r[4][slot], SB.r[5][slot]);
            }
            ps.pm = c3(1, 1, 1);
            ps.slot = slot;
            ps.depth = 0;
            ps.flags = 0;
            bump<ST>(c.samples);
            path_store<FRAY_SORT && sort_variant(ST)>(Q, slot, ps, ray_sort_class<ST>(ps.d, 0u));
        } else {
            PathRec* r = Q.rec + slot;
            r->d[0] = 0; r->d[1] = 0; r->d[2] = 0;
            r->depthFlags = FRAY_DEAD;
            if constexpr (FRAY_SORT && sort_variant(ST)) Q.cls[slot] = 15;
        }
        termCount[slot] = 0;
    }
    if (ST & 1) flush_stats(st, c);
}

struct WaveShare { uint32_t begin, end, chunk, w, W; };
FD WaveShare wave_share(uint32_t n)
{
    WaveShare r;
    r.W = gridDim.x * (blockDim.x >> 6);
    r.w = blockIdx.x * (blockDim.x >> 6) + (threadIdx.x >> 6);
    r.chunk = (((n + r.W - 1u) / r.W) + 63u) & ~63u;
    r.begin = r.w * r.chunk;
    r.end = r.begin + r.chunk < n ? r.begin + r.chunk : n;
    if (r.begin > n) r.begin = r.end = n;
    return r;
}


struct SegEnds { uint32_t begin, chunk, nF, nB; };
struct SegEndsShared { uint32_t begin, chunk; uint32_t* n; };
FD uint32_t seg_take(const SegEndsShared& E, bool back)
{
    const uint32_t k = atomicAdd(E.n + (back ? 1 : 0), 1u);
    return back ? E.begin + E.chunk - 1u - k : E.begin + k;
}
FD uint32_t seg_slot(const SegEnds& E, bool put, bool back)
{
    const uint32_t lane = threadIdx.x & 63u;
    const unsigned long long mF = __ballot(put && !back), mB = __ballot(put && back);
    const unsigned long long below = (1ull << lane) - 1ull;
    return back ? E.begin + E.chunk - 1u - (E.nB + (uint32_t)__popcll(mB & below)) : E.begin + E.nF + (uint32_t)__popcll(mF & below);
}
FD void seg_advance(SegEnds& E, bool put, bool back)
{
    E.nF += (uint32_t)__popcll(__ballot(put && !back));
    E.nB += (uint32_t)__popcll(__ballot(put && back));
}

template <int ST, bool BARY, class G>
FD void path_shade(const DScene& S, PathStateT<G>& ps, const HitT<ST>& h, const TermBuf& TB, DStats* st, const StereoBuf& SB, bool& cont, bool& shadow, uint32_t& shadowBack,
                   const ShadowQueue& SQ, const SegEndsShared& shadowEnds, Cnt& c)
{
    C3 own = c3(0, 0, 0);
    if (h.node <= -2) {
        own = (ps.flags & RF_DIFFUSE) ? c3(0, 0, 0) : light_color(S.lights[-2 - h.node]) * ps.pm;
        path_finish(TB, st, ps, SB);
    } else if (h.node < 0) {
        own = environment<ST>(S, ps.d, c) * ps.pm;
        path_finish(TB, st, ps, SB);
    } else {
        const FRAY_RO DNode& N = S.nodes[h.node];
        const FRAY_RO DShader& sh = S.shaders[N.shader];
        HitInfo info;
        finalize_hit<ST, BARY>(S, h, ps.o, ps.d, sh.usesUV || N.bumpTex >= 0, info);
        apply_bump<ST>(S, h.node, info, c);
        mt_skip(ps.tab, spawn_words(sh));
        {
            V3 sa, sb;
            C3 sc;
            shadow = nee_prepare(S, ps.d, info, ps.pm, sh, ps.rnd, ps.tab, sa, sb, sc, !(ST & 1) && S.skipNullSegments != 0);
            if (shadow) {
                bool planesPass = false;
                if constexpr (ST == 0 && FRAY_ARITH == 0) { if (S.certifiedSegments) planesPass = segment_certified(S, sa, sb); }
                shadowBack = ray_gate_class<tight_variant(ST)>(S, sa, sb - sa);
                if constexpr (ST == 0) {
                    if (FRAY_ARITH == 0 ? planesPass && shadowBack == 0 : segment_surely_visible(S, sa, sb, shadowBack)) {
                        own = sc;
                        shadow = false;
                        atomicAdd(shadowEnds.n + 2, 1u);
                    }
                }
                if (ST != 0 || shadow) {
                    const uint32_t j = seg_take(shadowEnds, shadowBack != 0);
                    SQ.ax[j] = sa.x; SQ.ay[j] = sa.y; SQ.az[j] = sa.z;
                    SQ.bx[j] = sb.x; SQ.by[j] = sb.y; SQ.bz[j] = sb.z;
                    SQ.cr[j] = sc.r; SQ.cg[j] = sc.g; SQ.cb[j] = sc.b;
                    SQ.slot[j] = ps.slot;
                    if constexpr (FRAY_SORT && sort_variant(ST)) SQ.cls[j] = (unsigned char)ray_sort_class<ST>(sb - sa, shadowBack);
                }
            }
        }
        PathRay win, wout;
        win.o = ps.o; win.d = ps.d; win.depth = ps.depth; win.flags = ps.flags;
        C3 brdf;
        float pdf;
        spawn_ray(sh, info, win, ps.tab, wout, brdf, pdf);
        {
            ps.pm = ps.pm * brdf / pdf;
            ps.o = wout.o; ps.d = wout.d; ps.depth = wout.depth; ps.flags = wout.flags;
#ifdef FRAY_SORT_BY_MATERIAL
            ps.flags = (ps.flags & 0xffu) | ((sh.kind == 1 ? 0u : sh.kind == 3 ? 1u : sh.kind == 4 ? 2u : 3u) << 8);
#endif
            if (ps.depth > S.maxTraceDepth || intensity(ps.pm) < 0.01) path_finish(TB, st, ps, SB);
            else cont = true;
        }
    }
    if (!shadow) term_store(TB, ps.slot, own);
}

struct LongRng { uint32_t* cols; uint32_t nPaths; DFrame F; int nItems, s0; };
struct FirstArgs { DCamera C; DFrame F; int nItems, s0; uint32_t n; const uint32_t* x397; unsigned short* termCount; };
struct BounceArgs { DScene S; PathQueue Qin, Qout; ShadowQueue SQ; QMetaRO metaIn; QMeta* metaOut; QMeta* metaShadow; TermBuf TB; StereoBuf SB; LongRng LR; DStats* st; FirstArgs FA; unsigned long long* segCertified; unsigned long long* camSkipped; };
#ifndef FRAY_ARITH
#define FRAY_ARITH 0
#endif
template <int ST, bool LONG, bool FIRST = false, int ARITH = FRAY_ARITH>
static __global__ __launch_bounds__(256, waves_for(ST, kd_variant(ST) ? FRAY_BOUNCE_WAVES : FRAY_BOUNCE_WAVES_NOKD)) void k_pt_bounce(BounceArgs A)
{
    static_assert(!(LONG && FIRST), "long generators start from k_pt_init");
    typedef typename std::conditional<LONG, MtPath, Mt>::type G;
    Cnt c = zero_cnt();
    const QMetaRO metaIn = A.metaIn;
    QMeta* const metaOut = A.metaOut;
    QMeta* const metaShadow = A.metaShadow;
    DStats* const st = A.st;
    const FRAY_RO uint32_t* off = FIRST ? nullptr : metaIn.p->off;
    const FRAY_RO uint32_t* nfIn = FIRST ? nullptr : metaIn.p->nf;
    const uint32_t nSeg = FIRST ? 1u : metaIn.p->nSeg, chunkIn = FIRST ? A.FA.n : metaIn.p->chunk;
    const bool certFront = !FIRST && metaIn.p->certFront != 0;
    const WaveShare ws = wave_share(FIRST ? A.FA.n : metaIn.p->n);
    const uint32_t lane = threadIdx.x & 63u;
    SegEnds outEnds{ws.begin, ws.chunk, 0, 0};
    __shared__ uint32_t shadowCount[4][ST == 0 ? 3 : 2];
    if (lane < (ST == 0 ? 3u : 2u)) shadowCount[threadIdx.x >> 6][lane] = 0;
    const SegEndsShared shadowEnds{ws.begin, ws.chunk, shadowCount[threadIdx.x >> 6]};
    uint32_t seg = (!FIRST && ws.begin < ws.end) ? seg_first(off, nSeg, ws.begin) : 0;
#ifdef FRAY_STAMPS
    stamp_begin();
#endif
    constexpr bool CAMSKIP = FIRST && tight_variant(ST);
    uint32_t camSkipped = 0, camWaves = 0;
    constexpr bool SORT = FRAY_SORT && !FIRST && sort_variant(ST);
    const uint32_t sortN = (uint32_t)FRAY_SORT_N;
    for (uint32_t b0 = ws.begin, b1 = 0; b0 < ws.end; b0 = b1) {
    b1 = (SORT && ws.end - b0 > sortN) ? b0 + sortN : ws.end;
    uint32_t* sorted = nullptr;
    if constexpr (SORT) {
        __shared__ uint32_t sortBuf[4][FRAY_SORT_N];
        __shared__ uint32_t sortCnt[4][16];
        sorted = sortBuf[threadIdx.x >> 6];
        const unsigned char* const cls = KARG(BounceArgs, kernel_args<BounceArgs>(), Qin).cls;
        sort_share(off, nfIn, nSeg, chunkIn, b0, b1, seg, sorted, sortCnt[threadIdx.x >> 6], [&](uint32_t i) { return (uint32_t)cls[i] & 15u; });
    }
    for (uint32_t base = b0; base < b1; base += 64u) {
        const FRAY_RO BounceArgs* AP = kernel_args<BounceArgs>();
        const FirstArgs& FA = KARG(BounceArgs, AP, FA);
        const DScene& S = KARG(BounceArgs, AP, S);
        const PathQueue& Qin = KARG(BounceArgs, AP, Qin);
        const PathQueue& Qout = KARG(BounceArgs, AP, Qout);
        const ShadowQueue& SQ = KARG(BounceArgs, AP, SQ);
        const TermBuf& TB = KARG(BounceArgs, AP, TB);
        const StereoBuf& SB = KARG(BounceArgs, AP, SB);
        const LongRng& LR = KARG(BounceArgs, AP, LR);
        const uint32_t di = base + lane;
        bool cont = false, shadow = false, gateFree = false;
        uint32_t shadowBack = 0;
        PathStateT<G> ps;
        if constexpr (CAMSKIP) { ps.o = v3(0, 0, 0); ps.d = v3(0, 0, 0); }
        bool live = di < b1;
        uint32_t i = di, seed0 = 0;
        if constexpr (FIRST) {
            if (live) {
                FA.termCount[di] = 0;
                int px, py;
                live = item_pixel(FA.F, (int)(di % (uint32_t)FA.nItems), px, py);
                if (live) {
                    seed0 = sample_seed(FA.F.seed, (uint32_t)py * (uint32_t)FA.F.W + (uint32_t)px, (uint32_t)(FA.s0 + (int)(di / (uint32_t)FA.nItems)));
                    Mt rnd = mt_seed_with(seed0, FA.x397[di]), tab = rnd;
                    const float ox = rng_float(rnd), oy = rng_float(rnd);
                    const double fx = (double)((float)px + ox), fy = (double)((float)py + oy);
                    if (FA.C.dof) dof_ray(FA.C, fx, fy, tab, ps.o, ps.d, 0); else screen_ray(FA.C, fx, fy, ps.o, ps.d, 0);
                }
            }
        } else {
            if constexpr (SORT) i = live ? sorted[di - b0] : 0u;
            else i = seg_map(off, nfIn, nSeg, chunkIn, base, di, live, seg);
            gateFree = certFront && (i & FRAY_FRONT_BIT);
            i &= ~FRAY_FRONT_BIT;
            if (live) {
                path_load_ray(Qin, i, ps);
                live = !(ps.d.x == 0 && ps.d.y == 0 && ps.d.z == 0);
            }
        }
        uint32_t skipNodes = 0;
        if constexpr (CAMSKIP) {
            if (S.nCamSkip > 0 && lanes(live) != 0) {
                skipNodes = camera_skip_nodes(S, ps.o, ps.d, live);
                camSkipped += (uint32_t)__builtin_popcount(skipNodes);
                camWaves++;
            }
        }
        if (live) {
            STAMP(0);
            HitT<ST> h;
            closest_hit<ST, CAMSKIP>(S, ps.o, ps.d, h, c, gateFree, skipNodes);
            if constexpr (FIRST) {
                ps.pm = c3(1, 1, 1); ps.slot = di; ps.depth = 0; ps.flags = 0;
                ps.rnd = mt_seed_with(seed0, FA.x397[di]);
                ps.tab = ps.rnd;
                mt_skip(ps.rnd, 2);
                if (FA.C.dof) mt_skip(ps.tab, 4);
                bump<ST>(c.samples);
            } else {
                path_load_rest(Qin, i, ps);
            }
#ifdef FRAY_QCHECK
            if (ps.slot >= TB.nPaths) { atomicAdd(&st->rngOverflow, 1ull << 32); ps.slot = 0; ps.pm = c3(0, 0, 0); ps.depth = 0x7fff; }
            else Qin.rec[i].slot = 0xffffffffu;
#endif
            if constexpr (LONG) {
                int px, py;
                item_pixel(LR.F, (int)(ps.slot % (uint32_t)LR.nItems), px, py);
                const uint32_t sd = sample_seed(LR.F.seed, (uint32_t)py * (uint32_t)LR.F.W + (uint32_t)px, (uint32_t)(LR.s0 + (int)(ps.slot / (uint32_t)LR.nItems)));
                ps.rnd.seed = ps.tab.seed = sd;
                ps.rnd.stride = ps.tab.stride = LR.nPaths;
                ps.rnd.col = LR.cols + ps.slot;
                ps.tab.col = LR.cols + (size_t)624 * LR.nPaths + ps.slot;
            }
            STAMP(8);
            path_shade<ST, false>(S, ps, h, TB, st, SB, cont, shadow, shadowBack, SQ, shadowEnds, c);
            STAMP(10);
        }
        const uint32_t gate = cont ? ray_gate_class<tight_variant(ST)>(S, ps.o, ps.d) : 0u;
        const bool back = gate != 0;
        const uint32_t slotOut = seg_slot(outEnds, cont, back);
#ifdef FRAY_SORT_BY_MATERIAL
        if (cont) path_store<true>(Qout, slotOut, ps, (ps.flags >> 8) & 3u);
#else
        if (cont) path_store<FRAY_SORT && sort_variant(ST)>(Qout, slotOut, ps, ray_sort_class<ST>(ps.d, gate));
#endif
        seg_advance(outEnds, cont, back);
        STAMP(13);
    }
    }
#ifdef FRAY_STAMPS
    if (lane < 24) { atomicAdd(&st->stamp[lane], g_stampAcc[threadIdx.x >> 6][lane]); atomicAdd(&st->stampLanes[lane], g_stampLanes[threadIdx.x >> 6][lane]); }
#endif
    if (lane == 0) {
        metaOut->cnt[ws.w] = outEnds.nF + outEnds.nB; metaOut->nf[ws.w] = outEnds.nF;
        metaShadow->cnt[ws.w] = shadowCount[threadIdx.x >> 6][0] + shadowCount[threadIdx.x >> 6][1]; metaShadow->nf[ws.w] = shadowCount[threadIdx.x >> 6][0];
        if constexpr (ST == 0) {
            unsigned long long* const total = KARG(BounceArgs, kernel_args<BounceArgs>(), segCertified);
            const uint32_t nCert = shadowCount[threadIdx.x >> 6][2];
            if (total && nCert) atomicAdd(total, (unsigned long long)nCert);
        }
        if constexpr (CAMSKIP) {
            unsigned long long* const pairs = KARG(BounceArgs, kernel_args<BounceArgs>(), camSkipped);
            if (pairs && camWaves) { atomicAdd(pairs, (unsigned long long)camSkipped); atomicAdd(pairs + 1, (unsigned long long)camWaves); }
        }
    }
    if (blockIdx.x == 0 && threadIdx.x == 0) {
        metaOut->chunk = ws.chunk; metaOut->nSeg = ws.W; metaShadow->chunk = ws.chunk; metaShadow->nSeg = ws.W;
        metaOut->certFront = metaShadow->certFront = A.S.gatesExact ? 1u : 0u;
    }
    if (ST & 1) flush_stats(st, c);
    if ((ST & 2) && c.envelope) atomicAdd(&st->rngOverflow, 1ull);
}

struct ShadowArgs { DScene S; ShadowQueue SQ; QMetaRO meta; TermBuf TB; DStats* st; unsigned long long* segSkipped; };
template <int ST, int ARITH = FRAY_ARITH>
static __global__ __launch_bounds__(256, anyhit_waves(ST)) void k_pt_shadow(ShadowArgs A)
{
    Cnt c = zero_cnt();
    const QMetaRO meta = A.meta;
    DStats* const st = A.st;
    const FRAY_RO uint32_t* off = meta.p->off;
    const FRAY_RO uint32_t* nfIn = meta.p->nf;
    const uint32_t nSeg = meta.p->nSeg, chunkIn = meta.p->chunk;
    const bool certFront = meta.p->certFront != 0;
    const WaveShare ws = wave_share(meta.p->n);
    const uint32_t lane = threadIdx.x & 63u;
    if (ws.begin >= ws.end) return;
    uint32_t seg = seg_first(off, nSeg, ws.begin);
#ifdef FRAY_STAMPS
    stamp_begin();
#endif
    constexpr bool SORT = FRAY_SORT && sort_variant(ST);
    constexpr bool SEGP = identity_variant(ST) && !(ST & 1);
// ... 170 lines not shown
```

### fray_amd/csrc/render_state.hpp

```cpp
#pragma once
#include <hip/hip_runtime.h>

#include <cstddef>
#include <string>
#include <vector>

#include "capi_common.h"
#include "dev_scene.hpp"
#include "dev_queues.hpp"

namespace frayhip_detail {
inline int hip_error_code(hipError_t e)
{
    switch (e) {
        case hipErrorOutOfMemory: return FRAYHIP_E_NOMEM;
        case hipErrorNoDevice: case hipErrorInvalidDevice: case hipErrorInsufficientDriver: case hipErrorNotInitialized: return FRAYHIP_E_NODEVICE;
        default: return FRAYHIP_E_HIP;
    }
}
}
#define HIP_TRY(expr)                                                                             \
    do {                                                                                          \
        hipError_t e_ = (expr);                                                                   \
        if (e_ != hipSuccess) {                                                                   \
            frayhip_detail::set_error(std::string(#expr) + ": " + hipGetErrorString(e_));         \
            return frayhip_detail::hip_error_code(e_);                                            \
        }                                                                                         \
    } while (0)

#ifndef FRAY_PT_BUDGET_MIB
#define FRAY_PT_BUDGET_MIB 24576
#endif
#ifndef FRAY_SEED_TABLE_MIB
#define FRAY_SEED_TABLE_MIB 4096
#endif
#ifndef FRAY_PT_LANES
#define FRAY_PT_LANES 4
#endif

struct SeedTable {
    uint32_t* d = nullptr;
    size_t bytes = 0;
    bool keyed = false;
    int32_t key[7] = {};
    uint32_t seed = 0;
    int nItems = 0;
    std::vector<unsigned char> valid;
    bool noGrow = false;
    bool serving = false;
};

struct SceneEdit;

struct frayhip_scene {
    void* d_arena = nullptr;
    size_t arena_bytes = 0;
    SceneEdit* edit = nullptr;
    long long sceneUpdates = 0, sceneUpdateBytes = 0;
    DScene S{};
    frayhip_camera camera{};
    frayhip_settings settings{};
    bool whittedNeedsRecursion = false;
    int specFanMax = 0;
    bool speculateFans = true;
    bool lightDraws = false;
    int lastWhittedPath = 0;
    int fusedWhittedMax = 4;
    int csgLanes = 1;
    unsigned warmMask = 0;
    bool fpContract = false;
    long long lastContracted = 0;
    bool skipNullSegments = true;
    bool segmentPlanes = true;
    bool certifiedSegments = true;
    bool tightGates = true;
    bool cameraSkip = true;
    long long lastCameraSkipped = 0, lastCameraWaves = 0;
    long long lastShadowCertified = 0;
    long long lastShadowNodesSkipped = 0;
    long long lastShadowSegments = 0;
    long long lastFans[4] = {0, 0, 0, 0};
    int lightSampleCount = 0;
    bool extGeometry = false;
    bool textured = false;
    bool kdMeshes = false;
    void* d_work = nullptr;
    size_t work_bytes = 0;
    DStats* d_stats = nullptr;
    void* d_motionTab = nullptr;
    size_t motionTabBytes = 0;
    std::vector<unsigned char> motionTabHost;
    QMeta* d_qmeta = nullptr;
    hipEvent_t evA = nullptr, evB = nullptr;
    std::vector<hipEvent_t> evPool, evPoolShadow;
    hipStream_t laneStream[FRAY_PT_LANES] = {};
    hipEvent_t evLaneStart = nullptr, evResolved[FRAY_PT_LANES] = {};
    int ptLanes = FRAY_PT_LANES;
    size_t ptBudgetBytes = (size_t)FRAY_PT_BUDGET_MIB << 20;
    size_t ptBudgetEff = 0;
    size_t seedTableCapBytes = (size_t)FRAY_SEED_TABLE_MIB << 20;
    SeedTable seedTab;
    int lastBatchLanes = 0;
    long long lastSeedLaunches = 0, lastSeedReused = 0;
    bool rendering = false;
};

namespace frayhip_detail {

constexpr size_t kSegTotalsOffset = 2 * sizeof(DStats);
constexpr size_t kSegSkippedOffset = kSegTotalsOffset + FRAY_PT_LANES * sizeof(unsigned long long);
constexpr size_t kSegCertifiedOffset = kSegSkippedOffset + FRAY_PT_LANES * sizeof(unsigned long long);
constexpr size_t kCamSkippedOffset = kSegCertifiedOffset + FRAY_PT_LANES * sizeof(unsigned long long);
constexpr size_t kCursorOffset = (kCamSkippedOffset + 2 * FRAY_PT_LANES * sizeof(unsigned long long) + 255) / 256 * 256;
constexpr size_t kStatsBytes = kCursorOffset + 3 * sizeof(DCursors);

DCamera camera_begin_frame(const frayhip_camera& c, int W, int H);
int persistent_grid(size_t n, int wavesPerSimd);
size_t work_budget(frayhip_scene* sc);
enum { FRAYHIP_RETRY_SMALLER = 1 };
int ensure_work_or_shrink(frayhip_scene* sc, size_t bytes, bool canRetry);
int bounce_grid(size_t n, bool alone);
int grid_for(size_t n);
int seed_grid(size_t n);
int ensure_work(frayhip_scene* sc, size_t bytes);
void seed_table_begin(frayhip_scene* sc, const DFrame& F, int nItems, int spp);
void seed_table_invalidate(frayhip_scene* sc);
void seed_table_free(frayhip_scene* sc);

struct Progress {
    const frayhip_progressive* req;
    float* h_rgb;
};
hipEvent_t pool_event(std::vector<hipEvent_t>& pool, size_t i);

}
```

### fray_amd/csrc/scene_arena.hpp

```cpp
#pragma once
#include <algorithm>
#include <cmath>
#include <cstddef>
#include <cstdint>
#include <cstring>
#include <functional>
#include <vector>

#include "dev_scene.hpp"

namespace frayhip_arena {

struct ArenaTable { uint64_t off, bytes; };

struct ArenaMeshTables { int32_t tris, attrs, kd, kdBox, refs, ltris, ltris32; };

struct ArenaFacts {
    int32_t extGeometry, kdMeshes, textured, whittedNeedsRecursion, lightDraws, lightSampleCount, specFanMax;
    int32_t nGates, gatesExact, nSegPlanes, nSegNodes, segCertAll;
    int32_t nTightGates;
    int32_t nCamSkip, tCamSkip;
    int32_t nNodes, nLights, nMeshes, nTextures;
    int32_t envPresent, envLoaded, envWidth[6], envHeight[6];
    int64_t envTexelOffset[6];
    int32_t tNodes, tNodesX, tGates, tSegPlanes, tSegMasks, tPlanes, tSpheres, tCubes, tCsgs, tTexels, tShaders, tLayers, tLights, tMeshes, tTex;
};

struct ArenaBuilt {
    std::vector<unsigned char> host;
    std::vector<ArenaTable> tables;
    std::vector<ArenaMeshTables> meshTables;
    std::vector<int64_t> texelOffset;
    ArenaFacts F;
};

namespace detail {

struct Arena {
    std::vector<unsigned char>& host;
    std::vector<ArenaTable>& tables;
    size_t add(const void* p, size_t bytes, size_t align = 256)
    {
        size_t off = (host.size() + align - 1) / align * align;
        host.resize(off + bytes);
        if (bytes) memcpy(host.data() + off, p, bytes);
        tables.push_back(ArenaTable{(uint64_t)off, (uint64_t)bytes});
        return off;
    }
    size_t reserve(size_t bytes)
    {
        size_t off = add(nullptr, 0);
        host.resize(off + bytes);
        tables.back().bytes = bytes;
        return off;
    }
    int32_t last() const { return (int32_t)tables.size() - 1; }
};

inline void put3(double* o, const double* p) { o[0] = p[0]; o[1] = p[1]; o[2] = p[2]; }
inline void putX(DXform& X, const frayhip_transform& T)
{
    put3(X.off, T.offset);
    memcpy(X.m, T.m, sizeof X.m);
    memcpy(X.inv, T.invM, sizeof X.inv);
}

inline bool shader_uses_uv(const frayhip_scene_desc& d, int s, int depth = 0)
{
    if (s < 0 || s >= d.n_shaders || depth > 40) return false;
    const frayhip_shader& sh = d.shaders[s];
    auto texUV = [&](int t) { return t >= 0 && t < d.n_textures && d.textures[t].kind != FRAYHIP_TEX_FRESNEL; };
    if (texUV(sh.texture)) return true;
    if (sh.kind == FRAYHIP_SHADER_LAYERED)
        for (int i = 0; i < sh.layer_count; i++) {
            const frayhip_layer& L = d.layers[sh.layer_begin + i];
            if (texUV(L.texture) || shader_uses_uv(d, L.shader, depth + 1)) return true;
        }
    return false;
}

inline bool arena_keeps_tris(const DMesh& M) { return !M.hasKd && M.nTris > 0 && M.nTris <= FRAY_GATECERT_MAX_TRIS; }
inline void fill_editable(const frayhip_scene_desc& d, const ArenaMeshTables* meshTables, ArenaFacts& F, unsigned char* const* tab)
{
    const DMesh* const meshes = (const DMesh*)tab[F.tMeshes];
    F.extGeometry = F.whittedNeedsRecursion = F.lightDraws = F.lightSampleCount = F.specFanMax = 0;
    for (int i = 0; i < d.n_nodes; i++) {
        int k = d.geoms[d.nodes[i].geom].kind;
        if (k == FRAYHIP_GEOM_CUBE || k == FRAYHIP_GEOM_CSG) F.extGeometry = 1;
    }
    std::vector<DNode> nodes(d.n_nodes);
    for (int i = 0; i < d.n_nodes; i++) {
        const frayhip_node& n = d.nodes[i];
        putX(nodes[i].T, n.T);
        nodes[i].geomKind = d.geoms[n.geom].kind;
        nodes[i].geomIndex = d.geoms[n.geom].index;
        nodes[i].shader = n.shader;
        nodes[i].bumpTex = n.bump_tex;
        nodes[i].xfClass = i;
        {
            static const double I9[9] = {1, 0, 0, 0, 1, 0, 0, 0, 1}, Z3[3] = {0, 0, 0};
            nodes[i].xfIdentity = (!memcmp(n.T.offset, Z3, sizeof Z3) && !memcmp(n.T.m, I9, sizeof I9) && !memcmp(n.T.invM, I9, sizeof I9)) ? 1 : 0;
        }
        for (int j = 0; j < i; j++)
            if (!memcmp(d.nodes[j].T.offset, n.T.offset, sizeof n.T.offset) && !memcmp(d.nodes[j].T.invM, n.T.invM, sizeof n.T.invM) &&
                !memcmp(d.nodes[j].T.m, n.T.m, sizeof n.T.m)) {
                nodes[i].xfClass = nodes[j].xfClass;
                break;
            }
        int sk = d.shaders[n.shader].kind;
        if (sk == FRAYHIP_SHADER_REFL || sk == FRAYHIP_SHADER_REFR || sk == FRAYHIP_SHADER_LAYERED) F.whittedNeedsRecursion = 1;
    }
    DPlane* const planes = (DPlane*)tab[F.tPlanes];
    for (int i = 0; i < d.n_planes; i++) { planes[i].limit = d.planes[i].limit; planes[i].height = d.planes[i].height; }
    DSphere* const spheres = (DSphere*)tab[F.tSpheres];
    for (int i = 0; i < d.n_spheres; i++) { put3(spheres[i].O, d.spheres[i].O); spheres[i].R = d.spheres[i].R; }
    DCube* const cubes = (DCube*)tab[F.tCubes];
    for (int i = 0; i < d.n_cubes; i++) { put3(cubes[i].O, d.cubes[i].O); cubes[i].halfSide = d.cubes[i].halfSide; }
    std::vector<DTexture> tex(d.n_textures);
    for (int i = 0; i < d.n_textures; i++) {
        const frayhip_texture& t = d.textures[i];
        DTexture& o = tex[i];
        o.kind = t.kind; o.width = t.width; o.height = t.height; o.pad = 0;
        memcpy(o.color1, t.color1, sizeof o.color1);
        memcpy(o.color2, t.color2, sizeof o.color2);
        o.scaling = t.scaling; o.bumpIntensity = t.bumpIntensity; o.ior = t.ior;
        o.texels = nullptr;
    }
    std::vector<DShader> shaders(d.n_shaders);
    for (int i = 0; i < d.n_shaders; i++) {
        const frayhip_shader& s = d.shaders[i];
        DShader& o = shaders[i];
        o.kind = s.kind; o.texture = s.texture;
        memcpy(o.color, s.color, sizeof o.color);
        memcpy(o.specularColor, s.specularColor, sizeof o.specularColor);
        memcpy(o.mult, s.mult, sizeof o.mult);
        o.numSamples = s.numSamples;
        o.exponent = s.exponent; o.specularMultiplier = s.specularMultiplier; o.glossiness = s.glossiness;
        o.deflectionScaling = s.deflectionScaling; o.ior = s.ior;
        o.layerBegin = s.layer_begin; o.layerCount = s.layer_count;
        o.usesUV = shader_uses_uv(d, i);
        o.pad = 0;
    }
    if (!shaders.empty()) memcpy(tab[F.tShaders], shaders.data(), shaders.size() * sizeof(DShader));
    std::vector<DLayer> layers(d.n_layers);
    for (int i = 0; i < d.n_layers; i++) {
        layers[i].shader = d.layers[i].shader; layers[i].texture = d.layers[i].texture;
        memcpy(layers[i].opacity, d.layers[i].opacity, sizeof layers[i].opacity);
        layers[i].pad = 0;
    }
    if (!layers.empty()) memcpy(tab[F.tLayers], layers.data(), layers.size() * sizeof(DLayer));
    std::vector<DLight> lights(d.n_lights);
    bool anyLightDraws = false;
    for (int i = 0; i < d.n_lights; i++) {
        const frayhip_light& l = d.lights[i];
        DLight& o = lights[i];
        o.kind = l.kind; o.xSubd = l.xSubd; o.ySubd = l.ySubd; o.pad = 0;
        memcpy(o.color, l.color, sizeof o.color);
        o.power = l.power;
        put3(o.pos, l.pos);
        putX(o.T, l.T);
        put3(o.center, l.center);
        o.area = l.area;
        F.lightSampleCount += l.kind == FRAYHIP_LIGHT_RECT ? l.xSubd * l.ySubd : 1;
        if (l.kind == FRAYHIP_LIGHT_RECT) F.lightDraws = 1;
        if (l.kind == FRAYHIP_LIGHT_RECT) anyLightDraws = true;
        o.areaXsize = 1.0 / l.xSubd;
        o.areaYsize = 1.0 / l.ySubd;
    }
    F.specFanMax = 0;
    if (!anyLightDraws)
        for (int i = 0; i < d.n_shaders; i++)
            if (d.shaders[i].kind == FRAYHIP_SHADER_REFL && d.shaders[i].glossiness != 1.0 && d.shaders[i].numSamples >= 8)
                F.specFanMax = std::max(F.specFanMax, (int)d.shaders[i].numSamples);
    if (!lights.empty()) memcpy(tab[F.tLights], lights.data(), lights.size() * sizeof(DLight));
    std::vector<DNodeX> nodesX(nodes.size());
    for (int i = 0; i < d.n_nodes; i++) {
        DNode& N = nodes[i];
        DNodeX& X = nodesX[i];
        N.tlTris = 0; N.tlCulling = 0; N.tlPtr = nullptr; N.boxMax = 0; N.gated = 0; N.segNode = 0;
        for (int k = 0; k < 3; k++) N.bmin[k] = N.bmax[k] = X.bminE[k] = X.bmaxE[k] = 0;
        if (N.geomKind == FRAYHIP_GEOM_MESH && !meshes[N.geomIndex].hasKd) {
            const DMesh& M = meshes[N.geomIndex];
            N.tlTris = M.nTris; N.tlCulling = M.culling;
            put3(N.bmin, M.bmin); put3(N.bmax, M.bmax);
            N.boxMax = M.boxMax;
            for (int k = 0; k < 3; k++) { X.bminE[k] = N.bmin[k] - 1e-6; X.bmaxE[k] = N.bmax[k] + 1e-6; }
        }
    }
    struct GB { bool ok; double lo[3], hi[3]; };
    std::function<GB(int, int)> bounds = [&](int g, int depth) -> GB {
        GB b{true, {0, 0, 0}, {0, 0, 0}};
        if (g < 0 || g >= d.n_geoms || depth > FRAY_CSG_DEPTH + 1) { b.ok = false; return b; }
        const int kind = d.geoms[g].kind, idx = d.geoms[g].index;
        if (kind == FRAYHIP_GEOM_PLANE) {
            b.ok = false; return b;
        } else if (kind == FRAYHIP_GEOM_SPHERE) {
            for (int k = 0; k < 3; k++) { b.lo[k] = d.spheres[idx].O[k] - std::fabs(d.spheres[idx].R); b.hi[k] = d.spheres[idx].O[k] + std::fabs(d.spheres[idx].R); }
        } else if (kind == FRAYHIP_GEOM_CUBE) {
            for (int k = 0; k < 3; k++) { b.lo[k] = d.cubes[idx].O[k] - std::fabs(d.cubes[idx].halfSide); b.hi[k] = d.cubes[idx].O[k] + std::fabs(d.cubes[idx].halfSide); }
        } else if (kind == FRAYHIP_GEOM_MESH) {
            for (int k = 0; k < 3; k++) { b.lo[k] = meshes[idx].bmin[k]; b.hi[k] = meshes[idx].bmax[k]; }
        } else if (kind == FRAYHIP_GEOM_CSG) {
            const frayhip_csg& C = d.csgs[idx];
            const GB L = bounds(C.left, depth + 1), R = bounds(C.right, depth + 1);
            auto vol = [](const GB& q) { return (q.hi[0] - q.lo[0]) * (q.hi[1] - q.lo[1]) * (q.hi[2] - q.lo[2]); };
            if (C.op == FRAYHIP_CSG_MINUS) return L;
            if (C.op == FRAYHIP_CSG_AND) { if (L.ok && R.ok) return vol(L) <= vol(R) ? L : R; return L.ok ? L : R; }
            if (!L.ok || !R.ok) { b.ok = false; return b; }
            for (int k = 0; k < 3; k++) { b.lo[k] = std::min(L.lo[k], R.lo[k]); b.hi[k] = std::max(L.hi[k], R.hi[k]); }
        } else b.ok = false;
        for (int k = 0; k < 3; k++) if (!(std::isfinite(b.lo[k]) && std::isfinite(b.hi[k]) && b.lo[k] <= b.hi[k])) b.ok = false;
        return b;
    };
    std::vector<GB> csgLocal(d.n_nodes, GB{false, {0, 0, 0}, {0, 0, 0}});
    for (int i = 0; i < d.n_nodes; i++) {
        DNodeX& X = nodesX[i];
        for (int k = 0; k < 3; k++) X.cc[k] = X.ch[k] = 0;
        X.cM = 0; X.csgBox = 0; X.padX = 0;
        if (nodes[i].geomKind != FRAYHIP_GEOM_CSG) continue;
        const GB b = bounds(d.nodes[i].geom, 0);
        if (!b.ok) continue;
        csgLocal[i] = b;
        for (int k = 0; k < 3; k++) {
            X.cc[k] = 0.5 * (b.lo[k] + b.hi[k]);
            X.ch[k] = std::max(b.hi[k] - X.cc[k], X.cc[k] - b.lo[k]) * (1.0 + 1e-12) + 1e-5;
            X.cM = std::max(X.cM, std::fabs(X.cc[k]) + X.ch[k]);
        }
        X.csgBox = X.cM < 1e9 ? 1 : 0;
    }
    int nSegPlanes = 0, nSegNodes = 0;
    {
        DSegPlane planes[FRAY_SEG_MAX_PLANES];
        double planeAmax[FRAY_SEG_MAX_PLANES];
        uint32_t masks[FRAY_SEG_MAX_NODES];
        int segNodeOf[FRAY_SEG_MAX_NODES];
        bool fits = true;
        for (int i = 0; i < d.n_nodes && fits; i++) {
            const DNode& N = nodes[i];
            if (!(N.tlTris > 0 && N.tlTris < FRAY_GATE_MIN_TRIS && N.xfIdentity)) continue;
// ... 33 lines not shown
    int nGates = 0, nTight = 0;
    bool gatesExact = false;
    {
        DGate gates[FRAY_MAX_GATES], tight[FRAY_MAX_GATES];
        int gateNode[FRAY_MAX_GATES];
        double smallest = 1e300;
        for (int i = 0; i < d.n_nodes; i++)
            if (csgLocal[i].ok) for (int k = 0; k < 3; k++) smallest = std::min(smallest, std::max(csgLocal[i].hi[k] - csgLocal[i].lo[k], 1e-9));
        for (int i = 0; i < d.n_nodes && nGates < FRAY_MAX_GATES; i++) {
            const DNode& N = nodes[i];
            double bmin[3], bmax[3];
            if (N.tlTris >= FRAY_GATE_MIN_TRIS) { put3(bmin, N.bmin); put3(bmax, N.bmax); }
            else if (csgLocal[i].ok) {
                bool huge = false;
                for (int k = 0; k < 3; k++) { bmin[k] = csgLocal[i].lo[k]; bmax[k] = csgLocal[i].hi[k]; huge = huge || bmax[k] - bmin[k] > 30.0 * smallest; }
                if (huge) continue;
            } else continue;
            DGate g;
            for (int k = 0; k < 3; k++) { g.lo[k] = 1e300; g.hi[k] = -1e300; }
            for (int c = 0; c < 8; c++) {
                const double p[3] = {c & 1 ? bmax[0] : bmin[0], c & 2 ? bmax[1] : bmin[1], c & 4 ? bmax[2] : bmin[2]};
                for (int k = 0; k < 3; k++) {
                    const double w = p[0] * N.T.m[k] + p[1] * N.T.m[3 + k] + p[2] * N.T.m[6 + k] + N.T.off[k];
                    g.lo[k] = std::min(g.lo[k], w); g.hi[k] = std::max(g.hi[k], w);
                }
            }
            g.exact = N.xfIdentity ? 1 : 0;
            g.Mf = 0;
            for (int k = 0; k < 3; k++) {
                const double c = 0.5 * (bmin[k] + bmax[k]), half = std::max(bmax[k] - c, c - bmin[k]);
                g.cf[k] = (float)c;
                g.hf[k] = std::nextafterf((float)(half * (1.0 + 1e-12) + 1e-5 + std::fabs(c - (double)g.cf[k])), INFINITY);
                g.Mf = std::max(g.Mf, std::nextafterf(std::fabs(g.cf[k]) + g.hf[k], INFINITY));
            }
            if (!(g.Mf < 1e9f)) g.exact = 0;
            g.guard = 0; g.nDirs = 0;
            for (int j = 0; j < FRAY_GATE_MAX_DIRS; j++) g.nf[j][0] = g.nf[j][1] = g.nf[j][2] = 0;
            for (int k = 0; k < 3; k++) { const double e = 1e-6 * (1.0 + std::fabs(g.lo[k]) + std::fabs(g.hi[k])); g.lo[k] -= e; g.hi[k] += e; }
            tight[nGates] = g;
            if (g.exact && N.tlTris >= FRAY_GATE_MIN_TRIS && N.tlTris <= FRAY_GATECERT_MAX_TRIS) {
                const DTri* const tris = (const DTri*)tab[meshTables[N.geomIndex].tris];
                GateTri gt[FRAY_GATECERT_MAX_TRIS];
                for (int t = 0; t < N.tlTris; t++) gt[t] = GateTri{tris[t].A, tris[t].AB, tris[t].AC, tris[t].N};
                DGateTight T;
                if (gatecert_make(T, gt, N.tlTris)) {
                    DGate& o = tight[nGates];
                    for (int k = 0; k < 3; k++) { o.cf[k] = T.cf[k]; o.hf[k] = T.hf[k]; }
                    o.Mf = T.Mf; o.guard = T.guard; o.nDirs = T.nDirs;
                    memcpy(o.nf, T.nf, sizeof o.nf);
                    nTight++;
                }
            }
            gateNode[nGates] = i;
            gates[nGates++] = g;
        }
        gatesExact = nGates > 0;
        for (int q = 0; q < nGates; q++) gatesExact = gatesExact && gates[q].exact;
        if (gatesExact)
            for (int q = 0; q < nGates; q++) nodes[gateNode[q]].gated = 1;
        memset(tab[F.tGates], 0, 2 * FRAY_MAX_GATES * sizeof(DGate));
        if (nGates) memcpy(tab[F.tGates], gates, (size_t)nGates * sizeof(DGate));
        if (nGates) memcpy(tab[F.tGates] + FRAY_MAX_GATES * sizeof(DGate), tight, (size_t)nGates * sizeof(DGate));
    }
    int nCamSkip = 0;
    {
        DCamSkip recs[FRAY_CAMSKIP_MAX];
        memset(recs, 0, sizeof recs);
        for (int i = 0; i < d.n_nodes && i < 32 && nCamSkip < FRAY_CAMSKIP_MAX; i++) {
            const DNode& N = nodes[i];
            if (!(N.tlTris > 0 && N.tlTris <= FRAY_GATECERT_MAX_TRIS && N.xfIdentity)) continue;
            const DTri* const tris = (const DTri*)tab[meshTables[N.geomIndex].tris];
            GateTri gt[FRAY_GATECERT_MAX_TRIS];
            for (int t = 0; t < N.tlTris; t++) gt[t] = GateTri{tris[t].A, tris[t].AB, tris[t].AC, tris[t].N};
            DGateTight T;
            if (!gatecert_make(T, gt, N.tlTris)) continue;
            DCamSkip& o = recs[nCamSkip++];
            for (int k = 0; k < 3; k++) { o.cf[k] = T.cf[k]; o.hf[k] = T.hf[k]; }
            o.Mf = T.Mf; o.guard = T.guard; o.nDirs = T.nDirs; o.node = i;
            memcpy(o.nf, T.nf, sizeof o.nf);
        }
        memcpy(tab[F.tCamSkip], recs, sizeof recs);
    }
    F.nCamSkip = nCamSkip;
    if (!nodes.empty()) memcpy(tab[F.tNodes], nodes.data(), nodes.size() * sizeof(DNode));
    if (!tex.empty()) memcpy(tab[F.tTex], tex.data(), tex.size() * sizeof(DTexture));

    F.nGates = nGates; F.gatesExact = gatesExact ? 1 : 0; F.nTightGates = nTight;
    F.nSegPlanes = nSegPlanes; F.nSegNodes = nSegNodes;
    bool segCertAll = true;
    for (int i = 0; i < d.n_nodes; i++) segCertAll = segCertAll && (nodes[i].segNode != 0 || nodes[i].gated != 0);
    segCertAll = segCertAll && d.n_lights > 0;
    const DSegPlane* const entries = (const DSegPlane*)tab[F.tSegPlanes];
    for (int p = 0; p < nSegPlanes && segCertAll; p++) {
        const DSegPlane& P = entries[p];
        bool off = false;
        for (int i = 0; i < d.n_lights && !off; i++) {
            const frayhip_light& l = d.lights[i];
            for (int c = 0; c < (l.kind == FRAYHIP_LIGHT_RECT ? 4 : 1) && !off; c++) {
                const double px = c & 1 ? 0.5 : -0.5, pz = c & 2 ? 0.5 : -0.5;
                double w[3];
                for (int k = 0; k < 3; k++) w[k] = l.kind == FRAYHIP_LIGHT_RECT ? px * l.T.m[k] + pz * l.T.m[6 + k] + l.T.offset[k] : l.pos[k];
                off = std::fabs(P.N[0] * w[0] + P.N[1] * w[1] + P.N[2] * w[2] - P.k) > P.t0;
            }
        }
        segCertAll = off;
    }
    const uint32_t* const nodeMasks = (const uint32_t*)tab[F.tSegMasks];
    bool starts = false;
    for (int j = 0; j < nSegNodes && !starts; j++) {
        bool clear = true;
        for (int p = 0; p < nSegPlanes; p++)
            if (nodeMasks[j] >> p & 1u) {
                const DSegPlane& P = entries[p];
                clear = clear && 1e-6 * std::sqrt(P.N[0] * P.N[0] + P.N[1] * P.N[1] + P.N[2] * P.N[2]) > P.t0;
            }
        starts = clear;
    }
    segCertAll = segCertAll && starts;
    F.segCertAll = segCertAll ? 1 : 0;
}

}

inline void arena_build(const frayhip_scene_desc& d, ArenaBuilt& B)
{
    using detail::put3;
    B.host.clear(); B.tables.clear(); B.meshTables.clear(); B.texelOffset.clear();
    ArenaFacts& F = B.F;
    memset(&F, 0, sizeof F);
    detail::Arena A{B.host, B.tables};
    A.reserve((size_t)d.n_nodes * sizeof(DNode));
    F.tNodes = A.last();
    A.reserve((size_t)d.n_nodes * sizeof(DNodeX));
    F.tNodesX = A.last();
    A.reserve(2 * FRAY_MAX_GATES * sizeof(DGate));
    F.tGates = A.last();
    A.reserve(FRAY_SEG_MAX_PLANES * sizeof(DSegPlane));
    F.tSegPlanes = A.last();
    A.reserve(FRAY_SEG_MAX_NODES * sizeof(uint32_t));
    F.tSegMasks = A.last();
    A.reserve((size_t)d.n_planes * sizeof(DPlane));
    F.tPlanes = A.last();
    A.reserve((size_t)d.n_spheres * sizeof(DSphere));
    F.tSpheres = A.last();
    A.reserve((size_t)d.n_cubes * sizeof(DCube));
    F.tCubes = A.last();
    std::vector<DCsg> csgs(d.n_csgs);
    for (int i = 0; i < d.n_csgs; i++) {
        const frayhip_csg& g = d.csgs[i];
        csgs[i].op = g.op;
        csgs[i].leftKind = d.geoms[g.left].kind; csgs[i].leftIndex = d.geoms[g.left].index; csgs[i].leftGeom = g.left;
        csgs[i].rightKind = d.geoms[g.right].kind; csgs[i].rightIndex = d.geoms[g.right].index; csgs[i].rightGeom = g.right;
        csgs[i].flat = (csgs[i].leftKind <= FRAYHIP_GEOM_CUBE && csgs[i].rightKind <= FRAYHIP_GEOM_CUBE) ? 1 : 0;
    }
    A.add(csgs.data(), csgs.size() * sizeof(DCsg));
    F.tCsgs = A.last();
    std::vector<DMesh> meshes(d.n_meshes);
    B.meshTables.resize(d.n_meshes);
    for (int mi = 0; mi < d.n_meshes; mi++) {
        const frayhip_mesh& m = d.meshes[mi];
        DMesh& M = meshes[mi];
        put3(M.bmin, m.bbox_min);
        put3(M.bmax, m.bbox_max);
        M.boxMax = 0;
        for (int k = 0; k < 3; k++) M.boxMax = std::max(M.boxMax, std::max(std::fabs(m.bbox_min[k]), std::fabs(m.bbox_max[k])));
        M.nTris = m.n_triangles;
        M.hasKd = m.has_kd;
        if (m.has_kd) F.kdMeshes = 1;
        M.smooth = !(m.faceted || m.n_normals == 0);
        M.culling = m.backfaceCulling;
        M.hasUV = m.n_uvs != 0;
        std::vector<DTri> tris(m.n_triangles);
        std::vector<DTriAttr> attrs(m.n_triangles);
        for (int t = 0; t < m.n_triangles; t++) {
            const frayhip_triangle& T = m.triangles[t];
            DTri& o = tris[t];
            put3(o.g, T.gnormal);
            put3(o.A, m.vertices + 3 * (size_t)T.v[0]);
            put3(o.N, T.ABcrossAC);
            put3(o.AC, T.AC);
            put3(o.AB, T.AB);
            o.index = t; o.pad = 0;
            DTriAttr& a = attrs[t];
            memset(&a, 0, sizeof a);
            if (M.smooth) {
                put3(a.nA, m.normals + 3 * (size_t)T.n[0]);
                put3(a.nB, m.normals + 3 * (size_t)T.n[1]);
                put3(a.nC, m.normals + 3 * (size_t)T.n[2]);
            }
            if (M.hasUV) {
                const double* tA = m.uvs + 3 * (size_t)T.t[0]; const double* tB = m.uvs + 3 * (size_t)T.t[1]; const double* tC = m.uvs + 3 * (size_t)T.t[2];
                a.tA[0] = tA[0]; a.tA[1] = tA[1]; a.tB[0] = tB[0]; a.tB[1] = tB[1]; a.tC[0] = tC[0]; a.tC[1] = tC[1];
            }
            put3(a.dNdx, T.dNdx);
            put3(a.dNdy, T.dNdy);
        }
        std::vector<DKd> kd(m.n_kdnodes);
        std::vector<DKdBox> kdBox(m.n_kdnodes);
        if (m.n_kdnodes > 0) {
            for (int k = 0; k < 3; k++) { kdBox[0].lo[k] = m.bbox_min[k]; kdBox[0].hi[k] = m.bbox_max[k]; }
            for (int n = 0; n < m.n_kdnodes; n++) {
                const frayhip_kdnode& K = m.kdnodes[n];
                DKd& o = kd[n];
                o.child0 = K.child0; o.meta = K.axis;
                if (K.axis != 3) {
                    o.split = K.split;
                    o.meta |= (m.kdnodes[K.child0].axis == 3 ? 4 : 0) | (m.kdnodes[K.child0 + 1].axis == 3 ? 8 : 0);
                    kdBox[K.child0] = kdBox[n];
                    kdBox[K.child0 + 1] = kdBox[n];
                    kdBox[K.child0].hi[K.axis] = K.split;
                    kdBox[K.child0 + 1].lo[K.axis] = K.split;
                } else {
                    o.triBegin = K.tri_begin; o.triCount = K.tri_count;
                }
            }
        }
        ArenaMeshTables& MT = B.meshTables[mi];
        A.add(tris.data(), tris.size() * sizeof(DTri)); MT.tris = A.last();
        A.add(attrs.data(), attrs.size() * sizeof(DTriAttr)); MT.attrs = A.last();
        A.add(kd.data(), kd.size() * sizeof(DKd)); MT.kd = A.last();
        A.add(kdBox.data(), kdBox.size() * sizeof(DKdBox)); MT.kdBox = A.last();
        A.add(m.trirefs, (size_t)m.n_trirefs * sizeof(int32_t)); MT.refs = A.last();
        std::vector<DTri> ltris((size_t)m.n_trirefs);
        for (int r = 0; r < m.n_trirefs; r++) ltris[r] = tris[m.trirefs[r]];
        A.add(ltris.data(), ltris.size() * sizeof(DTri)); MT.ltris = A.last();
        for (int k = 0; k < 3; k++) M.ref[k] = (m.bbox_min[k] + m.bbox_max[k]) * 0.5;
        std::vector<DTri32> l32(ltris.size());
        for (size_t r = 0; r < ltris.size(); r++) tricert_make(l32[r], ltris[r].A, ltris[r].AB, ltris[r].AC, ltris[r].N, M.ref);
        A.add(l32.data(), l32.size() * sizeof(DTri32)); MT.ltris32 = A.last();
    }
    A.add(d.texels, (size_t)d.n_texels * sizeof(float));
    F.tTexels = A.last();
    B.texelOffset.resize(d.n_textures);
    for (int i = 0; i < d.n_textures; i++) B.texelOffset[i] = d.textures[i].texel_offset;
    A.reserve((size_t)d.n_shaders * sizeof(DShader));
    F.tShaders = A.last();
    A.reserve((size_t)d.n_layers * sizeof(DLayer));
    F.tLayers = A.last();
    A.reserve((size_t)d.n_lights * sizeof(DLight));
    F.tLights = A.last();
    size_t oMeshes = A.reserve(meshes.size() * sizeof(DMesh));
    F.tMeshes = A.last();
    A.reserve((size_t)d.n_textures * sizeof(DTexture));
    F.tTex = A.last();
    if (!meshes.empty()) memcpy(A.host.data() + oMeshes, meshes.data(), meshes.size() * sizeof(DMesh));
    A.reserve(FRAY_CAMSKIP_MAX * sizeof(DCamSkip));
    F.tCamSkip = A.last();

    F.nNodes = d.n_nodes; F.nLights = d.n_lights; F.nMeshes = d.n_meshes; F.nTextures = d.n_textures;
    F.envPresent = d.environment.present;
    F.envLoaded = d.environment.loaded;
    if (d.n_textures > 0 || (d.environment.present && d.environment.loaded)) F.textured = 1;
    for (int f = 0; f < 6; f++) {
        F.envWidth[f] = d.environment.width[f];
        F.envHeight[f] = d.environment.height[f];
        F.envTexelOffset[f] = d.environment.texel_offset[f];
    }
    std::vector<unsigned char*> tab(B.tables.size());
    for (size_t t = 0; t < B.tables.size(); t++) tab[t] = B.host.data() + B.tables[t].off;
    detail::fill_editable(d, B.meshTables.data(), F, tab.data());
}

inline void arena_update(const frayhip_scene_desc& d, const ArenaMeshTables* meshTables, ArenaFacts& F, unsigned char* const* tab)
{
    detail::fill_editable(d, meshTables, F, tab);
}
inline void arena_update(const frayhip_scene_desc& d, ArenaBuilt& B)
{
    std::vector<unsigned char*> tab(B.tables.size());
    for (size_t t = 0; t < B.tables.size(); t++) tab[t] = B.host.data() + B.tables[t].off;
    arena_update(d, B.meshTables.data(), B.F, tab.data());
}
inline std::vector<int32_t> arena_editable_tables(const ArenaFacts& F)
{
    return {F.tNodes, F.tNodesX, F.tGates, F.tSegPlanes, F.tSegMasks, F.tPlanes, F.tSpheres, F.tCubes, F.tShaders, F.tLayers, F.tLights, F.tTex, F.tCamSkip};
}

inline void arena_place(const ArenaFacts& F, const ArenaMeshTables* meshTables, const int64_t* texelOffset, unsigned char* const* write,
                        const unsigned char* const* addr, DScene& S)
{
    DMesh* const meshes = (DMesh*)write[F.tMeshes];
    for (int mi = 0; mi < F.nMeshes; mi++) {
        const ArenaMeshTables& MT = meshTables[mi];
        meshes[mi].tris = (const FRAY_RO DTri*)addr[MT.tris];
        meshes[mi].attrs = (const FRAY_RO DTriAttr*)addr[MT.attrs];
        meshes[mi].kd = (const FRAY_RO DKd*)addr[MT.kd];
        meshes[mi].kdBox = (const FRAY_RO DKdBox*)addr[MT.kdBox];
        meshes[mi].refs = (const FRAY_RO int32_t*)addr[MT.refs];
        meshes[mi].ltris = (const FRAY_RO DTri*)addr[MT.ltris];
        meshes[mi].ltris32 = (const FRAY_RO DTri32*)addr[MT.ltris32];
    }
    DNode* const nodes = (DNode*)write[F.tNodes];
    for (int i = 0; i < F.nNodes; i++)
        if (nodes[i].geomKind == FRAYHIP_GEOM_MESH && !meshes[nodes[i].geomIndex].hasKd) nodes[i].tlPtr = meshes[nodes[i].geomIndex].tris;
    DTexture* const tex = (DTexture*)write[F.tTex];
    for (int i = 0; i < F.nTextures; i++) tex[i].texels = (const FRAY_RO float*)addr[F.tTexels] + texelOffset[i];

    S.nodes = (const FRAY_RO DNode*)addr[F.tNodes];
    S.nodesX = (const FRAY_RO DNodeX*)addr[F.tNodesX];
    S.gates = (const FRAY_RO DGate*)addr[F.tGates];
    S.nGates = F.nGates; S.gatesExact = F.gatesExact;
    S.segPlanes = (const FRAY_RO DSegPlane*)addr[F.tSegPlanes];
    S.segNodeMasks = (const FRAY_RO uint32_t*)addr[F.tSegMasks];
    S.nSegPlanes = F.nSegPlanes; S.nSegNodes = F.nSegNodes; S.segCertAll = F.segCertAll;
    S.camSkip = (const FRAY_RO DCamSkip*)addr[F.tCamSkip];
    S.nCamSkip = F.nCamSkip; S.padCamSkip = 0;
    S.planes = (const FRAY_RO DPlane*)addr[F.tPlanes];
    S.spheres = (const FRAY_RO DSphere*)addr[F.tSpheres];
    S.cubes = (const FRAY_RO DCube*)addr[F.tCubes];
    S.csgs = (const FRAY_RO DCsg*)addr[F.tCsgs];
    S.meshes = (const FRAY_RO DMesh*)addr[F.tMeshes];
    S.shaders = (const FRAY_RO DShader*)addr[F.tShaders];
    S.layers = (const FRAY_RO DLayer*)addr[F.tLayers];
    S.textures = (const FRAY_RO DTexture*)addr[F.tTex];
    S.lights = (const FRAY_RO DLight*)addr[F.tLights];
    S.env.present = F.envPresent;
    S.env.loaded = F.envLoaded;
    for (int f = 0; f < 6; f++) {
        S.env.width[f] = F.envWidth[f];
        S.env.height[f] = F.envHeight[f];
        S.env.face[f] = (const FRAY_RO float*)addr[F.tTexels] + F.envTexelOffset[f];
    }
    S.nNodes = F.nNodes;
    S.nLights = F.nLights;
    S.probPickLight = F.nLights > 0 ? 1.0f / (float)F.nLights : 0.0f;
}

}
```

### fray_amd/scene.py

```python
import ctypes as C
import math
import os
import sys

import numpy as np

from . import abi

P = C.POINTER

_HERE = os.path.dirname(os.path.abspath(__file__))
_LIB_PATH = os.environ.get("FRAYHIP_LIB") or os.path.join(_HERE, "libfrayhip.so")


class FrayError(RuntimeError):
    def __init__(self, code, msg):
        super().__init__("frayhip error %d: %s" % (code, msg))
        self.code = code


def _load():
    if "torch" not in sys.modules and not os.environ.get("FRAYHIP_NO_TORCH"):
        try:
            import torch
# ... 605 lines not shown
    def __init__(self):
        self._hs = C.c_void_p()
        self._dev = C.c_void_p()
        self.desc = None

    @classmethod
    def parseScene(cls, path):
        s = cls()
        _check(lib.frayhip_scene_parse(os.fspath(path).encode(), C.byref(s._hs)))
        s.desc = lib.frayhip_host_scene_desc(s._hs).contents
        return s

    @property
    def settings(self):
        return self.desc.settings

    @property
    def camera(self):
        return self.desc.camera

    def _table(self, name, rec):
        n = getattr(self.desc, "n_" + name)
        return C.cast(getattr(self.desc, name), P(rec * n)).contents if n else (rec * 0)()

    nodes = property(lambda self: self._table("nodes", abi.Node), doc="desc.nodes[] as a mutable array of abi.Node")
    lights = property(lambda self: self._table("lights", abi.Light), doc="desc.lights[] (abi.Light)")
    shaders = property(lambda self: self._table("shaders", abi.Shader), doc="desc.shaders[] (abi.Shader)")
    layers = property(lambda self: self._table("layers", abi.Layer), doc="desc.layers[] (abi.Layer)")
    textures = property(lambda self: self._table("textures", abi.Texture), doc="desc.textures[] (abi.Texture): color1, color2, scaling, bumpIntensity and ior are editable")
    spheres = property(lambda self: self._table("spheres", abi.Sphere), doc="desc.spheres[] (abi.Sphere)")
    planes = property(lambda self: self._table("planes", abi.Plane), doc="desc.planes[] (abi.Plane)")
    cubes = property(lambda self: self._table("cubes", abi.Cube), doc="desc.cubes[] (abi.Cube)")

    @property
    def frame_size(self):
        return self.desc.settings.frameWidth, self.desc.settings.frameHeight

    def samples_per_pixel(self):
        spp = 5 if self.settings.wantAA else 1
        if self.camera.dof:
            spp = max(spp, self.camera.numDOFSamples)
        if self.settings.gi:
            spp = max(spp, self.settings.numPaths)
        return spp

    def beginRender(self, device=None):
        if device is not None:
            _check(lib.frayhip_init(int(device)))
        self.endRender()
        _check(lib.frayhip_scene_create(C.byref(self.desc), C.byref(self._dev)))
        return self

    def beginFrame(self):
        self._need_dev()
        _check(lib.frayhip_scene_set_view(self._dev, C.byref(self.desc.camera), C.byref(self.desc.settings)))
        return self

    def update(self):
        self._need_dev()
        _check(lib.frayhip_scene_update(self._dev, C.byref(self.desc)))
        return self

    def endRender(self):
        if self._dev:
            lib.frayhip_scene_destroy(self._dev)
            self._dev = C.c_void_p()

    def set_option(self, name, value):
        self._need_dev()
        _check(lib.frayhip_scene_set_option(self._dev, name.encode(), int(value)))
        return self

    def tight_gates(self, enable=None):
        self._need_dev()
        on, n = C.c_int64(0), C.c_int64(0)
        _check(lib.frayhip_scene_tight_gates(self._dev, -1 if enable is None else int(bool(enable)), C.byref(on), C.byref(n)))
        return int(on.value), int(n.value)

    def camera_skip(self, enable=None):
        self._need_dev()
        on, n, skipped, waves = C.c_int64(0), C.c_int64(0), C.c_int64(0), C.c_int64(0)
        _check(lib.frayhip_scene_camera_skip(self._dev, -1 if enable is None else int(bool(enable)), C.byref(on), C.byref(n), C.byref(skipped), C.byref(waves)))
        return int(on.value), int(n.value), int(skipped.value), int(waves.value)

    def get_option(self, name):
        self._need_dev()
        v = C.c_int64(0)
        _check(lib.frayhip_scene_get_option(self._dev, name.encode(), C.byref(v)))
        return int(v.value)

    def _frame(self, mode, seed, bucket_first, bucket_stride, spp_chunk, stats):
        return abi.Frame(mode=mode, seed=seed, bucket_first=bucket_first, bucket_stride=bucket_stride,
                         spp_chunk=spp_chunk, flags=abi.FRAME_STATS if stats else 0)

    def _need_dev(self):
        if not self._dev:
            raise FrayError(abi.E_ARG, "Scene.beginRender() has not been called")

    def render(self, seed=42, bucket_first=0, bucket_stride=1, spp_chunk=0, stats=False, out=None, progress=None, preview_ms=-1):
        self._need_dev()
        W, H = self.frame_size
        rgb = out if out is not None else np.zeros((H, W, 3), np.float32)
        st = abi.Stats()
        fr = self._frame(abi.MODE_RENDER, seed, bucket_first, bucket_stride, spp_chunk, stats)
        if progress is None:
            _check(lib.frayhip_render(self._dev, C.byref(fr), rgb.ctypes.data, None, None, C.byref(st)))
            return rgb, st.as_dict()
        req, run = _progress_request(progress, preview_ms, lambda p: {"image": np.ctypeslib.as_array(p.rgb, shape=(H, W, 3))})
        rc = lib.frayhip_render_progressive(self._dev, C.byref(fr), C.byref(req), rgb.ctypes.data, None, None, C.byref(st))
        return rgb, run.finish(rc, st)

    def primary_hits(self, bucket_first=0, bucket_stride=1, stats=False):
        self._need_dev()
        W, H = self.frame_size
        ids = np.full((H, W), -9, np.int32)
        dist = np.zeros((H, W), np.float64)
        st = abi.Stats()
        fr = self._frame(abi.MODE_PRIMARY_ID, 0, bucket_first, bucket_stride, 0, stats)
        _check(lib.frayhip_render(self._dev, C.byref(fr), None, ids.ctypes.data, dist.ctypes.data, C.byref(st)))
        return ids, dist, st.as_dict()

    def render_device(self, d_rgb_ptr, seed=42, bucket_first=0, bucket_stride=1, spp_chunk=0, stats=False,
                      stream=None, mode=abi.MODE_RENDER, d_id_ptr=None, d_dist_ptr=None, progress=None, preview_ms=-1):
        self._need_dev()
        st = abi.Stats()
        fr = self._frame(mode, seed, bucket_first, bucket_stride, spp_chunk, stats)
        if progress is None:
            _check(lib.frayhip_render_device(self._dev, C.byref(fr), d_rgb_ptr, d_id_ptr, d_dist_ptr, stream, C.byref(st)))
            return st.as_dict()
        req, run = _progress_request(progress, preview_ms, lambda p: {"d_rgb": C.cast(p.rgb, C.c_void_p).value})
        rc = lib.frayhip_render_device_progressive(self._dev, C.byref(fr), C.byref(req), d_rgb_ptr, d_id_ptr, d_dist_ptr, stream, C.byref(st))
        return run.finish(rc, st)

    def camera_rays(self, xy=None, eye=0, stream=None):
        self._need_dev()
        if xy is None:
            W, H = self.frame_size
            org, dirs = np.empty((H, W, 3)), np.empty((H, W, 3))
            _check(lib.frayhip_camera_rays(self._dev, W * H, None, int(eye), org.ctypes.data, dirs.ctypes.data))
            return org, dirs
        (xy,), shape, device = _query_inputs([("xy", xy)], 2)
        n = int(np.prod(shape, dtype=np.int64))
        if device is None:
            xy = np.ascontiguousarray(xy)
            org, dirs = np.empty(shape + (3,)), np.empty(shape + (3,))
            _check(lib.frayhip_camera_rays(self._dev, n, xy.ctypes.data, int(eye), org.ctypes.data, dirs.ctypes.data))
            return org, dirs
        with _DeviceCall(device, stream) as call:
            torch = call.torch
            xy = xy.contiguous()
            org = torch.empty(shape + (3,), dtype=torch.float64, device=device)
            dirs = torch.empty(shape + (3,), dtype=torch.float64, device=device)
            if n:
                _check(lib.frayhip_camera_rays_device(self._dev, n, xy.data_ptr(), int(eye), org.data_ptr(), dirs.data_ptr(), call.handle))
        return org, dirs

    def trace_rays(self, origin, dir, record=False, stats=False, stream=None):
        self._need_dev()
        (o, d), shape, device = _query_inputs([("origin", origin), ("dir", dir)])
        n = int(np.prod(shape, dtype=np.int64))
        st = abi.Stats()
        flags = abi.FRAME_STATS if stats else 0
        if device is None:
            o, d = np.ascontiguousarray(o), np.ascontiguousarray(d)
            ids, dist = np.empty(shape, np.int32), np.empty(shape, np.float64)
            rec = np.empty(shape + (9,), np.float64) if record else None
# ... 570 lines not shown
```

### include/frayhip.h

```cpp
#ifndef FRAYHIP_H
#define FRAYHIP_H

#include <stdint.h>

#ifdef __cplusplus
extern "C" {
#endif

#define FRAYHIP_ABI_VERSION 3

enum {
    FRAYHIP_OK            = 0,
    FRAYHIP_E_ARG         = -1,
    FRAYHIP_E_PARSE       = -2,
    FRAYHIP_E_NODEVICE    = -3,
    FRAYHIP_E_UNSUPPORTED = -4,
    FRAYHIP_E_NOMEM       = -5,
    FRAYHIP_E_HIP         = -6,
    FRAYHIP_E_CANCELLED   = -7,
};


typedef struct frayhip_transform {
    double offset[3];
// ... 115 lines not shown
    const frayhip_geom_ref* geoms;
    const frayhip_plane*    planes;
    const frayhip_sphere*   spheres;
    const frayhip_cube*     cubes;
    const frayhip_csg*      csgs;
    const frayhip_mesh*     meshes;
    const frayhip_shader*   shaders;
    const frayhip_layer*    layers;
    const frayhip_texture*  textures;
    const frayhip_light*    lights;
    const float*            texels;
    frayhip_environment environment;
    frayhip_camera      camera;
    frayhip_settings    settings;
} frayhip_scene_desc;

enum {
    FRAYHIP_MODE_PRIMARY_ID = 0,
    FRAYHIP_MODE_RENDER     = 1,
};

#define FRAYHIP_BUCKET_SKEW 3
typedef struct frayhip_frame {
    int32_t  mode;
    uint32_t seed;
    int32_t  bucket_first, bucket_stride;
    int32_t  spp_chunk;
    int32_t  flags;
} frayhip_frame;

enum {
    FRAYHIP_FRAME_STATS = 1,
};

typedef struct frayhip_stats {
    uint64_t closest_rays;
    uint64_t shadow_rays;
    uint64_t node_tests;
    uint64_t kd_inner_visits;
    uint64_t leaf_refs;
    uint64_t tri_tests;
    uint64_t prim_tests;
    uint64_t smooth_hits;
    uint64_t samples;
    uint64_t texture_fetches;
    double   ms_total;
    double   ms_kernels;
    double   ms_trace;
    uint64_t trace_launches;
    double   alg_bytes_trace;
    double   ms_shadow;
    uint64_t shadow_launches;
    double   alg_bytes_shadow;
    double   alg_flops_trace;
    double   alg_flops_shadow;
} frayhip_stats;

typedef struct frayhip_host_scene frayhip_host_scene;

int  frayhip_scene_parse(const char* fray_path, frayhip_host_scene** out);
frayhip_scene_desc* frayhip_host_scene_desc(frayhip_host_scene* hs);
void frayhip_host_scene_free(frayhip_host_scene* hs);

typedef struct frayhip_scene frayhip_scene;

int  frayhip_init(int device_id);
int  frayhip_scene_create(const frayhip_scene_desc* desc, frayhip_scene** out);
void frayhip_scene_destroy(frayhip_scene* s);
int  frayhip_scene_set_view(frayhip_scene* s, const frayhip_camera* camera, const frayhip_settings* settings);

int  frayhip_scene_update(frayhip_scene* s, const frayhip_scene_desc* desc);

int  frayhip_transform_identity(frayhip_transform* T);
int  frayhip_transform_scale(frayhip_transform* T, double x, double y, double z);
int  frayhip_transform_rotate(frayhip_transform* T, double yaw, double pitch, double roll);
int  frayhip_transform_translate(frayhip_transform* T, double x, double y, double z);
int  frayhip_light_begin_frame(frayhip_light* light);
int  frayhip_shader_begin_frame(frayhip_shader* shader);

int  frayhip_scene_set_option(frayhip_scene* s, const char* name, int64_t value);
int  frayhip_scene_get_option(frayhip_scene* s, const char* name, int64_t* value);
int  frayhip_scene_tight_gates(frayhip_scene* s, int enable, int64_t* enabled, int64_t* eligible);
int  frayhip_scene_camera_skip(frayhip_scene* s, int enable, int64_t* enabled, int64_t* eligible, int64_t* skipped, int64_t* waves);

int  frayhip_render(frayhip_scene* s, const frayhip_frame* f,
                    float* rgb, int32_t* hit_id, double* hit_dist, frayhip_stats* st);
int  frayhip_render_device(frayhip_scene* s, const frayhip_frame* f,
                           float* d_rgb, int32_t* d_hit_id, double* d_hit_dist,
                           void* hip_stream, frayhip_stats* st);

typedef struct frayhip_progress {
    int32_t samples_done;
    int32_t samples_total;
    int32_t batches_done, batches_total;
    double  ms_elapsed;
    int32_t preview;
    int32_t final;
    const float* rgb;
} frayhip_progress;

typedef struct frayhip_progressive {
    int  (*fn)(void* user, const frayhip_progress* p);
    void*  user;
    double preview_ms;
} frayhip_progressive;

int  frayhip_render_progressive(frayhip_scene* s, const frayhip_frame* f, const frayhip_progressive* p,
                                float* rgb, int32_t* hit_id, double* hit_dist, frayhip_stats* st);
int  frayhip_render_device_progressive(frayhip_scene* s, const frayhip_frame* f, const frayhip_progressive* p,
                                       float* d_rgb, int32_t* d_hit_id, double* d_hit_dist, void* hip_stream, frayhip_stats* st);

int  frayhip_camera_rays(frayhip_scene* s, int64_t n, const double* xy, int eye, double* origin, double* dir);
int  frayhip_camera_rays_device(frayhip_scene* s, int64_t n, const double* d_xy, int eye,
                                double* d_origin, double* d_dir, void* hip_stream);
int  frayhip_trace_rays(frayhip_scene* s, int64_t n, const double* origin, const double* dir, int flags,
                        int32_t* hit_id, double* hit_dist, double* hit_rec, frayhip_stats* st);
int  frayhip_trace_rays_device(frayhip_scene* s, int64_t n, const double* d_origin, const double* d_dir, int flags,
                               int32_t* d_hit_id, double* d_hit_dist, double* d_hit_rec, void* hip_stream, frayhip_stats* st);
int  frayhip_visible(frayhip_scene* s, int64_t n, const double* a, const double* b, int flags, uint8_t* vis, frayhip_stats* st);
int  frayhip_visible_device(frayhip_scene* s, int64_t n, const double* d_a, const double* d_b, int flags,
                            uint8_t* d_vis, void* hip_stream, frayhip_stats* st);

typedef struct frayhip_shade_request {
    uint32_t seed;
    int32_t  spp;
    int32_t  sample_first;
    int32_t  rng_skip;
    int32_t  flags;
    int32_t  _pad;
    const uint32_t* keys;
} frayhip_shade_request;

int  frayhip_shade_rays(frayhip_scene* s, int64_t n, const double* origin, const double* dir,
                        const frayhip_shade_request* r, float* rgb, frayhip_stats* st);
int  frayhip_shade_rays_device(frayhip_scene* s, int64_t n, const double* d_origin, const double* d_dir,
                               const frayhip_shade_request* r, float* d_rgb, void* hip_stream, frayhip_stats* st);

typedef struct frayhip_adaptive {
    int32_t  min_spp;
    int32_t  _pad;
    double   threshold;
    double   err_floor;
    int32_t  rungs;
    int32_t  _pad2;
    uint64_t samples;
} frayhip_adaptive;

int  frayhip_render_adaptive(frayhip_scene* s, const frayhip_frame* f, frayhip_adaptive* a,
                             float* rgb, int32_t* spp_out, float* err_out, frayhip_stats* st);
int  frayhip_render_device_adaptive(frayhip_scene* s, const frayhip_frame* f, frayhip_adaptive* a,
                                    float* d_rgb, int32_t* d_spp, float* d_err, void* hip_stream, frayhip_stats* st);

#define FRAYHIP_ACCUM_CHANNELS 4
typedef struct frayhip_samples {
    int32_t sample_first;
    int32_t sample_count;
    int32_t samples_done;
    int32_t _pad;
} frayhip_samples;

int  frayhip_render_samples(frayhip_scene* s, const frayhip_frame* f, frayhip_samples* r, const frayhip_progressive* p,
                            float* accum, float* rgb, float* noise, frayhip_stats* st);
int  frayhip_render_samples_device(frayhip_scene* s, const frayhip_frame* f, frayhip_samples* r, const frayhip_progressive* p,
                                   float* d_accum, float* d_rgb, float* d_noise, void* hip_stream, frayhip_stats* st);

int  frayhip_render_components(frayhip_scene* s, const frayhip_frame* f, frayhip_samples* r, const frayhip_progressive* p,
// ... 182 lines not shown
```

Measured before the change: 14030.

## Add shading shortcuts: precomputed world normals, diagonal light transforms, shift subdivisions

Adds a scene-specialized shading path for non-textured variants. When every node is an identity-transform flat mesh, finalize_hit reads a host-precomputed per-triangle world normal table instead of recomputing geometry. For rect lights with purely diagonal transforms, the matrix multiplies in sampling and light intersection are replaced with per-axis scaling. Power-of-two subdivisions use mask/shift instead of div/mod. It costs extra arena memory for the normal table and more template variants, and the diagonal check rejects lights with zero offsets by default.

```diff
diff --git a/fray_amd/abi.py b/fray_amd/abi.py
--- a/fray_amd/abi.py
+++ b/fray_amd/abi.py
@@ -243,6 +243,7 @@
     "frayhip_scene_get_option": (C.c_int, [VP, C.c_char_p, P(i64)]),
     "frayhip_scene_tight_gates": (C.c_int, [VP, C.c_int, P(i64), P(i64)]),
     "frayhip_scene_camera_skip": (C.c_int, [VP, C.c_int, P(i64), P(i64), P(i64), P(i64)]),
+    "frayhip_scene_shade_shortcuts": (C.c_int, [VP, C.c_int, P(i64), P(i64)]),
     "frayhip_render": (C.c_int, [VP, P(Frame), VP, VP, VP, P(Stats)]),
     "frayhip_render_device": (C.c_int, [VP, P(Frame), VP, VP, VP, VP, P(Stats)]),
     "frayhip_render_progressive": (C.c_int, [VP, P(Frame), P(Progressive), VP, VP, VP, P(Stats)]),
diff --git a/fray_amd/csrc/capi.hip b/fray_amd/csrc/capi.hip
--- a/fray_amd/csrc/capi.hip
+++ b/fray_amd/csrc/capi.hip
@@ -254,6 +254,7 @@
     S.segmentPlanes = s->segmentPlanes ? 1 : 0;
     S.certifiedSegments = (s->certifiedSegments && s->segmentPlanes && S.segCertAll) ? 1 : 0;
     if (!s->cameraSkip) S.nCamSkip = 0;
+    if (!s->shadeShortcuts) S.shadeIdentity = S.lightsDiagonal = S.subdShift = 0;
     return S;
 }
 
@@ -588,6 +589,7 @@
     if (const char* e = getenv("FRAYHIP_CERTIFIED_SEGMENTS")) sc->certifiedSegments = atol(e) != 0;
     if (const char* e = getenv("FRAYHIP_TIGHT_GATES")) sc->tightGates = atol(e) != 0;
     if (const char* e = getenv("FRAYHIP_CAMERA_SKIP")) sc->cameraSkip = atol(e) != 0;
+    if (const char* e = getenv("FRAYHIP_SHADE_SHORTCUTS")) sc->shadeShortcuts = atol(e) != 0;
     if (const char* e = getenv("FRAYHIP_FUSED_WHITTED_MAX")) { long v = atol(e); if (v >= 0 && v <= 1024) sc->fusedWhittedMax = (int)v; }
     if (const char* e = getenv("FRAYHIP_CSG_LANES")) { long v = atol(e); if (v >= 1 && v <= FRAY_PT_LANES) sc->csgLanes = (int)v; }
     if (const char* e = getenv("FRAYHIP_SEED_TABLE_MIB")) { long v = atol(e); if (v >= 0 && v <= (1 << 20)) sc->seedTableCapBytes = (size_t)v << 20; }
@@ -697,6 +699,17 @@
     return FRAYHIP_OK;
 }
 
+int frayhip_scene_shade_shortcuts(frayhip_scene* s, int enable, int64_t* enabled, int64_t* eligible)
+{
+    if (!s) { set_error("frayhip_scene_shade_shortcuts: null scene"); return FRAYHIP_E_ARG; }
+    if (enable < -1 || enable > 1) { set_error("frayhip_scene_shade_shortcuts: enable must be -1, 0 or 1"); return FRAYHIP_E_ARG; }
+    if (enable >= 0 && s->rendering) { set_error("frayhip_scene_shade_shortcuts: the scene is rendering a frame"); return FRAYHIP_E_ARG; }
+    if (enable >= 0) s->shadeShortcuts = enable != 0;
+    if (enabled) *enabled = s->shadeShortcuts ? 1 : 0;
+    if (eligible) *eligible = (s->edit->F.shadeIdentity ? 1 : 0) | (s->edit->F.lightsDiagonal ? 2 : 0);
+    return FRAYHIP_OK;
+}
+
 int frayhip_scene_set_view(frayhip_scene* s, const frayhip_camera* camera, const frayhip_settings* settings)
 {
     if (!s) { set_error("frayhip_scene_set_view: null scene"); return FRAYHIP_E_ARG; }
diff --git a/fray_amd/csrc/dev_scene.hpp b/fray_amd/csrc/dev_scene.hpp
--- a/fray_amd/csrc/dev_scene.hpp
+++ b/fray_amd/csrc/dev_scene.hpp
@@ -105,7 +105,8 @@
 struct DLayer { int32_t shader, texture; float opacity[3]; int32_t pad; };
 
 struct DLight {
-    int32_t kind, xSubd, ySubd, pad;
+    int32_t kind, xSubd, ySubd;
+    int32_t xShift;
     float color[3], power;
     double pos[3];
     DXform T;
@@ -164,6 +165,9 @@
     int32_t certifiedSegments;
     const FRAY_RO DCamSkip* camSkip;
     int32_t nCamSkip, padCamSkip;
+    const FRAY_RO double* worldNormals;
+    int32_t normStride, shadeIdentity, lightsDiagonal;
+    int32_t subdShift;
 };
 
 struct DFrame {
diff --git a/fray_amd/csrc/dev_shade.hpp b/fray_amd/csrc/dev_shade.hpp
--- a/fray_amd/csrc/dev_shade.hpp
+++ b/fray_amd/csrc/dev_shade.hpp
@@ -3,6 +3,10 @@
 #include "dev_rng.hpp"
 #include "dev_scene.hpp"
 #include "dev_trace.hpp"
+
+#ifndef FRAY_SHADE_PLUS_ZERO
+#define FRAY_SHADE_PLUS_ZERO 1
+#endif
 
 enum { RF_DIFFUSE = 2 };
 
@@ -51,9 +55,21 @@
     }
 }
 
-template <int ST, bool BARY = false, bool ANY_UV = false>
+template <int ST, bool BARY = false, bool ANY_UV = false, bool SHORTCUT = false>
 FD void finalize_hit(const DScene& S, const HitT<ST>& h, V3 o, V3 d, bool needUV, HitInfo& info)
 {
+    if constexpr (SHORTCUT) {
+        info.dNdx = v3(0, 0, 0);
+        info.dNdy = v3(0, 0, 0);
+        info.u = 0; info.v = 0;
+        if (S.shadeIdentity) {
+            const V3 ldir = normalized(d);
+            const V3 ipl = o + ldir * h.t;
+            info.ip = FRAY_SHADE_PLUS_ZERO ? ipl + v3(0.0, 0.0, 0.0) : ipl;
+            info.norm = ld3(S.worldNormals + 3 * (h.node * S.normStride + h.tri));
+            return;
+        }
+    }
     const FRAY_RO DNode& N = S.nodes[h.node];
     needUV = needUV && (ANY_UV || tex_variant(ST));
     const bool needBump = tex_variant(ST) && N.bumpTex >= 0;
@@ -183,16 +199,22 @@
 
 FD int light_num_samples(const FRAY_RO DLight& L) { return L.kind == 0 ? 1 : L.xSubd * L.ySubd; }
 FD C3 light_color(const FRAY_RO DLight& L) { return ldc(L.color) * L.power; }
-template <class G>
-FD void light_nth_sample(const FRAY_RO DLight& L, int idx, V3 shadePos, G& tab, V3& samplePos, C3& color)
+template <bool SHORTCUT = false, class G>
+FD void light_nth_sample(const FRAY_RO DLight& L, int idx, V3 shadePos, G& tab, V3& samplePos, C3& color, bool diagonal = false, bool shift = false)
 {
     if (L.kind == 0) {
         samplePos = ld3(L.pos);
         color = ldc(L.color) * L.power;
         return;
     }
-    int col = idx % L.xSubd;
-    int row = idx / L.xSubd;
+    int col, row;
+    if (SHORTCUT && shift && L.xShift >= 0) {
+        col = idx & (L.xSubd - 1);
+        row = idx >> L.xShift;
+    } else {
+        col = idx % L.xSubd;
+        row = idx / L.xSubd;
+    }
     double cellW = L.areaXsize;
     double cellH = L.areaYsize;
     double x0 = col * cellW;
@@ -200,14 +222,18 @@
     double p_x = x0 + cellW * rng_float(tab);
     double p_y = y0 + cellH * rng_float(tab);
     V3 pl = v3(p_x - 0.5, 0, p_y - 0.5);
-    V3 sp = mulM(shadePos - ld3(L.T.off), L.T.inv);
+    const V3 rel = shadePos - ld3(L.T.off);
+    V3 sp;
+    if (SHORTCUT && diagonal) sp = v3(rel.x * L.T.inv[0], rel.y * L.T.inv[4], rel.z * L.T.inv[8]);
+    else sp = mulM(rel, L.T.inv);
     if (sp.y > 0) {
         color = c3(0, 0, 0);
     } else {
         float cw = float(fray_div(dot(v3(0, -1, 0), sp), length(sp)));
         color = ldc(L.color) * L.power * (float)L.area * cw;
     }
-    samplePos = mulM(pl, L.T.m) + ld3(L.T.off);
+    if (SHORTCUT && diagonal) samplePos = v3(pl.x * L.T.m[0] + L.T.off[0], L.T.off[1], pl.z * L.T.m[8] + L.T.off[2]);
+    else samplePos = mulM(pl, L.T.m) + ld3(L.T.off);
 }
 FD double light_solid_angle(const FRAY_RO DLight& L, V3 ip)
 {
@@ -329,7 +355,7 @@
     pdf = 1;
 }
 
-template <class GR, class GT>
+template <bool SHORTCUT = false, class GR, class GT>
 FD bool nee_prepare(const DScene& S, V3 rayDir, const HitInfo& info, C3 pm, const FRAY_RO DShader& sh, GR& rnd, GT& tab, V3& a, V3& b, C3& contrib, bool skipNull)
 {
     if (S.nLights == 0) return false;
@@ -341,7 +367,7 @@
     int randSample = rng_int0(rnd, light_num_samples(L) - 1);
     V3 pl;
     C3 unused;
-    light_nth_sample(L, randSample, x, tab, pl, unused);
+    light_nth_sample<SHORTCUT>(L, randSample, x, tab, pl, unused, SHORTCUT && S.lightsDiagonal != 0, SHORTCUT && S.subdShift != 0);
     if (skipNull && (sh.kind == 3 || sh.kind == 4)) return false;
     a = x + info.norm * 1e-6;
     b = pl;
diff --git a/fray_amd/csrc/dev_trace.hpp b/fray_amd/csrc/dev_trace.hpp
--- a/fray_amd/csrc/dev_trace.hpp
+++ b/fray_amd/csrc/dev_trace.hpp
@@ -25,6 +25,7 @@
 constexpr bool tex_variant(int st) { return (st & 14) != 0; }
 constexpr bool identity_variant(int st) { return FRAY_IDENTITY_SKIP && (st & 14) == 0; }
 constexpr bool tight_variant(int st) { return FRAY_ARITH == 0 && (st & 15) == 0; }
+constexpr bool shade_shortcut_variant(int st) { return identity_variant(st) && !(st & 1); }
 
 struct HitRec {
     int node;
@@ -844,13 +845,20 @@
     return true;
 }
 
-template <int ST>
-FD bool light_intersect(const FRAY_RO DLight& L, V3 o, V3 d, double& dist, Cnt& c)
+template <int ST, bool SHORTCUT = false>
+FD bool light_intersect(const FRAY_RO DLight& L, V3 o, V3 d, double& dist, Cnt& c, bool diagonal = false)
 {
     if (L.kind == 0) return false;
     bump<ST>(c.prim);
-    V3 ls = mulM(o - ld3(L.T.off), L.T.inv);
-    V3 ldir = normalized(mulM(d, L.T.inv));
+    const V3 rel = o - ld3(L.T.off);
+    V3 ls, ldir;
+    if (SHORTCUT && diagonal) {
+        ls = v3(rel.x * L.T.inv[0], rel.y * L.T.inv[4], rel.z * L.T.inv[8]);
+        ldir = normalized(v3(d.x * L.T.inv[0], d.y * L.T.inv[4], d.z * L.T.inv[8]));
+    } else {
+        ls = mulM(rel, L.T.inv);
+        ldir = normalized(mulM(d, L.T.inv));
+    }
     if (ls.y >= 0) return false;
     if (ldir.y <= 0) return false;
     double travelByY = fabs(ls.y);
@@ -858,7 +866,8 @@
     double scaling = fray_div(travelByY, unitTravel);
     V3 ip = ls + ldir * scaling;
     if (fabs(ip.x) > 0.5 || fabs(ip.z) > 0.5) return false;
-    ip = mulM(ip, L.T.m) + ld3(L.T.off);
+    if (SHORTCUT && diagonal) ip = v3(ip.x * L.T.m[0], ip.y * L.T.m[4], ip.z * L.T.m[8]) + ld3(L.T.off);
+    else ip = mulM(ip, L.T.m) + ld3(L.T.off);
     dist = length(o - ip);
     return true;
 }
@@ -872,7 +881,7 @@
     norm = normalized(mulM(v3(0, -1, 0), L.T.m));
 }
 
-template <int ST, bool CAMSKIP = false>
+template <int ST, bool CAMSKIP = false, bool SHORTCUT = false>
 FD void closest_hit(const DScene& S, V3 o, V3 d, HitT<ST>& best, Cnt& c, bool gateFree = false, uint32_t skipNodes = 0u)
 {
     bump<ST>(c.closest);
@@ -908,7 +917,7 @@
     const int nl = S.nLights;
     for (int i = 0; i < nl; i++) {
         double dist;
-        if (light_intersect<ST>(S.lights[i], o, d, dist, c) && dist < best.dist) {
+        if (light_intersect<ST, SHORTCUT>(S.lights[i], o, d, dist, c, SHORTCUT && S.lightsDiagonal != 0) && dist < best.dist) {
             best.node = -2 - i;
             best.dist = dist;
         }
diff --git a/fray_amd/csrc/kernels.hpp b/fray_amd/csrc/kernels.hpp
--- a/fray_amd/csrc/kernels.hpp
+++ b/fray_amd/csrc/kernels.hpp
@@ -950,13 +950,13 @@
         const FRAY_RO DNode& N = S.nodes[h.node];
         const FRAY_RO DShader& sh = S.shaders[N.shader];
         HitInfo info;
-        finalize_hit<ST, BARY>(S, h, ps.o, ps.d, sh.usesUV || N.bumpTex >= 0, info);
+        finalize_hit<ST, BARY, false, shade_shortcut_variant(ST)>(S, h, ps.o, ps.d, sh.usesUV || N.bumpTex >= 0, info);
         apply_bump<ST>(S, h.node, info, c);
         mt_skip(ps.tab, spawn_words(sh));
         {
             V3 sa, sb;
             C3 sc;
-            shadow = nee_prepare(S, ps.d, info, ps.pm, sh, ps.rnd, ps.tab, sa, sb, sc, !(ST & 1) && S.skipNullSegments != 0);
+            shadow = nee_prepare<shade_shortcut_variant(ST)>(S, ps.d, info, ps.pm, sh, ps.rnd, ps.tab, sa, sb, sc, !(ST & 1) && S.skipNullSegments != 0);
             if (shadow) {
                 bool planesPass = false;
                 if constexpr (ST == 0 && FRAY_ARITH == 0) { if (S.certifiedSegments) planesPass = segment_certified(S, sa, sb); }
@@ -1091,7 +1091,7 @@
         if (live) {
             STAMP(0);
             HitT<ST> h;
-            closest_hit<ST, CAMSKIP>(S, ps.o, ps.d, h, c, gateFree, skipNodes);
+            closest_hit<ST, CAMSKIP, shade_shortcut_variant(ST)>(S, ps.o, ps.d, h, c, gateFree, skipNodes);
             if constexpr (FIRST) {
                 ps.pm = c3(1, 1, 1); ps.slot = di; ps.depth = 0; ps.flags = 0;
                 ps.rnd = mt_seed_with(seed0, FA.x397[di]);
diff --git a/fray_amd/csrc/render_state.hpp b/fray_amd/csrc/render_state.hpp
--- a/fray_amd/csrc/render_state.hpp
+++ b/fray_amd/csrc/render_state.hpp
@@ -75,6 +75,7 @@
     bool certifiedSegments = true;
     bool tightGates = true;
     bool cameraSkip = true;
+    bool shadeShortcuts = true;
     long long lastCameraSkipped = 0, lastCameraWaves = 0;
     long long lastShadowCertified = 0;
     long long lastShadowNodesSkipped = 0;
diff --git a/fray_amd/csrc/scene_arena.hpp b/fray_amd/csrc/scene_arena.hpp
--- a/fray_amd/csrc/scene_arena.hpp
+++ b/fray_amd/csrc/scene_arena.hpp
@@ -20,6 +20,8 @@
     int32_t nGates, gatesExact, nSegPlanes, nSegNodes, segCertAll;
     int32_t nTightGates;
     int32_t nCamSkip, tCamSkip;
+    int32_t shadeIdentity, lightsDiagonal;
+    int32_t normStride, tWorldNormals;
     int32_t nNodes, nLights, nMeshes, nTextures;
     int32_t envPresent, envLoaded, envWidth[6], envHeight[6];
     int64_t envTexelOffset[6];
@@ -79,6 +81,25 @@
     return false;
 }
 
+inline void world_normal(const double* g, const double* m, double* out)
+{
+    const double x = g[0] * m[0] + g[1] * m[3] + g[2] * m[6], y = g[0] * m[1] + g[1] * m[4] + g[2] * m[7], z = g[0] * m[2] + g[1] * m[5] + g[2] * m[8];
+    const double r = 1.0 / std::sqrt(x * x + y * y + z * z);
+    out[0] = x * r; out[1] = y * r; out[2] = z * r;
+}
+#ifndef FRAY_LIGHT_ZERO_OFFSET_OK
+#define FRAY_LIGHT_ZERO_OFFSET_OK 0
+#endif
+inline bool light_is_diagonal(const frayhip_light& l)
+{
+    bool ok = l.kind == FRAYHIP_LIGHT_RECT;
+    for (int k = 0; k < 9; k++) {
+        const bool diag = k == 0 || k == 4 || k == 8;
+        ok = ok && (diag ? std::isfinite(l.T.m[k]) && std::isfinite(l.T.invM[k]) : l.T.m[k] == 0.0 && l.T.invM[k] == 0.0);
+    }
+    for (int k = 0; k < 3; k++) ok = ok && std::isfinite(l.T.offset[k]) && (FRAY_LIGHT_ZERO_OFFSET_OK || l.T.offset[k] != 0.0);
+    return ok;
+}
 inline bool arena_keeps_tris(const DMesh& M) { return !M.hasKd && M.nTris > 0 && M.nTris <= FRAY_GATECERT_MAX_TRIS; }
 inline void fill_editable(const frayhip_scene_desc& d, const ArenaMeshTables* meshTables, ArenaFacts& F, unsigned char* const* tab)
 {
@@ -154,7 +175,10 @@
     for (int i = 0; i < d.n_lights; i++) {
         const frayhip_light& l = d.lights[i];
         DLight& o = lights[i];
-        o.kind = l.kind; o.xSubd = l.xSubd; o.ySubd = l.ySubd; o.pad = 0;
+        o.kind = l.kind; o.xSubd = l.xSubd; o.ySubd = l.ySubd;
+        o.xShift = -1;
+        if (l.kind == FRAYHIP_LIGHT_RECT && l.xSubd > 0 && (l.xSubd & (l.xSubd - 1)) == 0)
+            for (o.xShift = 0; (1 << o.xShift) < l.xSubd;) o.xShift++;
         memcpy(o.color, l.color, sizeof o.color);
         o.power = l.power;
         put3(o.pos, l.pos);
@@ -354,6 +378,27 @@
         memcpy(tab[F.tCamSkip], recs, sizeof recs);
     }
     F.nCamSkip = nCamSkip;
+    {
+        const size_t entries = (size_t)d.n_nodes * (size_t)F.normStride;
+        double* const wn = (double*)tab[F.tWorldNormals];
+        if (entries) memset(wn, 0, entries * 3 * sizeof(double));
+        bool all = entries > 0;
+        for (int i = 0; i < d.n_nodes && entries; i++) {
+            const DNode& N = nodes[i];
+            bool ok = N.xfIdentity && N.geomKind == FRAYHIP_GEOM_MESH && N.bumpTex < 0 && !shaders[N.shader].usesUV;
+            if (ok) { const DMesh& M = meshes[N.geomIndex]; ok = arena_keeps_tris(M) && !M.smooth && M.nTris <= F.normStride; }
+            all = all && ok;
+            if (!ok) continue;
+            const DTri* const tris = (const DTri*)tab[meshTables[N.geomIndex].tris];
+            for (int t = 0; t < meshes[N.geomIndex].nTris; t++) world_normal(tris[t].g, N.T.m, wn + 3 * ((size_t)i * F.normStride + t));
+        }
+        F.shadeIdentity = all ? 1 : 0;
+    }
+    {
+        bool all = d.n_lights > 0;
+        for (int i = 0; i < d.n_lights; i++) all = all && light_is_diagonal(d.lights[i]);
+        F.lightsDiagonal = all ? 1 : 0;
+    }
     if (!nodes.empty()) memcpy(tab[F.tNodes], nodes.data(), nodes.size() * sizeof(DNode));
     if (!tex.empty()) memcpy(tab[F.tTex], tex.data(), tex.size() * sizeof(DTexture));
 
@@ -518,6 +563,9 @@
     if (!meshes.empty()) memcpy(A.host.data() + oMeshes, meshes.data(), meshes.size() * sizeof(DMesh));
     A.reserve(FRAY_CAMSKIP_MAX * sizeof(DCamSkip));
     F.tCamSkip = A.last();
+    F.normStride = d.n_nodes <= 4096 ? FRAY_GATECERT_MAX_TRIS : 0;
+    A.reserve((size_t)d.n_nodes * (size_t)F.normStride * 3 * sizeof(double));
+    F.tWorldNormals = A.last();
 
     F.nNodes = d.n_nodes; F.nLights = d.n_lights; F.nMeshes = d.n_meshes; F.nTextures = d.n_textures;
     F.envPresent = d.environment.present;
@@ -545,7 +593,7 @@
 }
 inline std::vector<int32_t> arena_editable_tables(const ArenaFacts& F)
 {
-    return {F.tNodes, F.tNodesX, F.tGates, F.tSegPlanes, F.tSegMasks, F.tPlanes, F.tSpheres, F.tCubes, F.tShaders, F.tLayers, F.tLights, F.tTex, F.tCamSkip};
+    return {F.tNodes, F.tNodesX, F.tGates, F.tSegPlanes, F.tSegMasks, F.tPlanes, F.tSpheres, F.tCubes, F.tShaders, F.tLayers, F.tLights, F.tTex, F.tCamSkip, F.tWorldNormals};
 }
 
 inline void arena_place(const ArenaFacts& F, const ArenaMeshTables* meshTables, const int64_t* texelOffset, unsigned char* const* write,
@@ -577,6 +625,8 @@
     S.nSegPlanes = F.nSegPlanes; S.nSegNodes = F.nSegNodes; S.segCertAll = F.segCertAll;
     S.camSkip = (const FRAY_RO DCamSkip*)addr[F.tCamSkip];
     S.nCamSkip = F.nCamSkip; S.padCamSkip = 0;
+    S.worldNormals = (const FRAY_RO double*)addr[F.tWorldNormals];
+    S.normStride = F.normStride; S.shadeIdentity = F.shadeIdentity; S.lightsDiagonal = F.lightsDiagonal; S.subdShift = 1;
     S.planes = (const FRAY_RO DPlane*)addr[F.tPlanes];
     S.spheres = (const FRAY_RO DSphere*)addr[F.tSpheres];
     S.cubes = (const FRAY_RO DCube*)addr[F.tCubes];
diff --git a/fray_amd/scene.py b/fray_amd/scene.py
--- a/fray_amd/scene.py
+++ b/fray_amd/scene.py
@@ -711,6 +711,12 @@
         on, n, skipped, waves = C.c_int64(0), C.c_int64(0), C.c_int64(0), C.c_int64(0)
         _check(lib.frayhip_scene_camera_skip(self._dev, -1 if enable is None else int(bool(enable)), C.byref(on), C.byref(n), C.byref(skipped), C.byref(waves)))
         return int(on.value), int(n.value), int(skipped.value), int(waves.value)
+
+    def shade_shortcuts(self, enable=None):
+        self._need_dev()
+        on, el = C.c_int64(0), C.c_int64(0)
+        _check(lib.frayhip_scene_shade_shortcuts(self._dev, -1 if enable is None else int(bool(enable)), C.byref(on), C.byref(el)))
+        return int(on.value), int(el.value)
 
     def get_option(self, name):
         self._need_dev()
diff --git a/include/frayhip.h b/include/frayhip.h
--- a/include/frayhip.h
+++ b/include/frayhip.h
@@ -221,6 +221,7 @@
 int  frayhip_scene_get_option(frayhip_scene* s, const char* name, int64_t* value);
 int  frayhip_scene_tight_gates(frayhip_scene* s, int enable, int64_t* enabled, int64_t* eligible);
 int  frayhip_scene_camera_skip(frayhip_scene* s, int enable, int64_t* enabled, int64_t* eligible, int64_t* skipped, int64_t* waves);
+int  frayhip_scene_shade_shortcuts(frayhip_scene* s, int enable, int64_t* enabled, int64_t* eligible);
 
 int  frayhip_render(frayhip_scene* s, const frayhip_frame* f,
                     float* rgb, int32_t* hit_id, double* hit_dist, frayhip_stats* st);
```

Result: faster. 14380, median of 6 (+2.5%).
